# shenyunhang/APE

Measured on AMD Instinct MI355X. Metric: images/sec @1024^2 APE-L_D fwd, higher is better.
Workload: dtype bf16

## Files before the change

ape_amd/_lib.py:

```python
import ctypes
import os
from ctypes import POINTER, Structure, c_char_p, c_double, c_float, c_int, c_int32, c_int64, c_void_p

_HERE = os.path.dirname(os.path.abspath(__file__))
LIB_PATH = os.path.join(_HERE, "lib", "libape_hip.so")

DT_F32 = 0
DT_BF16 = 1
DT_F16 = 2
ACT_NONE, ACT_RELU, ACT_GELU, ACT_SWIGLU, ACT_SILU = 0, 1, 2, 3, 4
MASK_NONE, MASK_ZERO_INPUT, MASK_ZERO_OUTPUT = 0, 1, 2


class GemmArgs(Structure):
    _fields_ = [
        ("A", c_void_p), ("W", c_void_p), ("C", c_void_p), ("bias", c_void_p), ("residual", c_void_p),
        ("rowmask", c_void_p), ("rope_cos", c_void_p), ("rope_sin", c_void_p),
        ("M", c_int32), ("N", c_int32), ("K", c_int32),
        ("lda", c_int32), ("ldw", c_int32), ("ldc", c_int32), ("ldr", c_int32),
        ("in_dt", c_int32), ("out_dt", c_int32), ("res_dt", c_int32),
        ("act", c_int32), ("mask_mode", c_int32), ("trans_out", c_int32),
        ("rope_rows", c_int32), ("rope_hd", c_int32), ("rope_cols", c_int32), ("vec_ok", c_int32),
        ("alpha", c_float), ("clamp", c_float),
        ("splitk", c_int32), ("tile64", c_int32), ("workspace", c_void_p),
        ("rowscale", c_void_p), ("rowshift", c_void_p), ("colvec", c_void_p), ("rope_cs", c_void_p),
        ("ln_w", c_void_p), ("ln_b", c_void_p), ("ln_eps", c_float), ("reserved0", c_int32),
        ("conv_perm", c_void_p), ("conv_zero", c_void_p), ("conv_h", c_int32), ("conv_w", c_int32),
        ("rowstat_cols", c_int32), ("rowstat_eps", c_float),
    ]


class LayerNormArgs(Structure):
    _fields_ = [
        ("x", c_void_p), ("w", c_void_p), ("b", c_void_p), ("y", c_void_p), ("add", c_void_p), ("y2", c_void_p),
        ("M", c_int32), ("C", c_int32), ("Cpad", c_int32),
        ("ldx", c_int32), ("ldy", c_int32), ("ldadd", c_int32), ("ldy2", c_int32),
        ("x_dt", c_int32), ("y_dt", c_int32), ("add_dt", c_int32), ("act", c_int32), ("eps", c_float),
    ]


class GroupNormArgs(Structure):
    _fields_ = [
        ("x", c_void_p), ("w", c_void_p), ("b", c_void_p), ("y", c_void_p), ("add", c_void_p), ("workspace", c_void_p),
        ("HW", c_int32), ("C", c_int32), ("G", c_int32),
        ("ldx", c_int32), ("ldy", c_int32), ("ldadd", c_int32),
        ("x_dt", c_int32), ("y_dt", c_int32), ("add_dt", c_int32), ("act", c_int32), ("eps", c_float),
    ]


SIGNATURES = {
    "ape_hip_last_error": (c_char_p, []),
    "ape_hip_abi_version": (c_int, []),
    "ape_hip_sizeof_args": (c_int, [c_int]),
    "ape_hip_gemm": (c_int, [POINTER(GemmArgs), c_void_p]),
    "ape_hip_gemm_last_kernel": (c_char_p, []),
    "ape_hip_meter_begin": (c_int, []),
    "ape_hip_meter_count": (c_int, []),
    "ape_hip_meter_end": (c_int, []),
    "ape_hip_meter_read": (c_int, [c_int, POINTER(c_char_p), POINTER(c_float)]),
    "ape_hip_zero": (c_int, [c_void_p, ctypes.c_size_t, c_void_p]),
    "ape_hip_stuff_collapse": (c_int, [c_void_p, c_int, c_int, c_int, c_int, c_void_p, c_int, c_void_p]),
    "ape_hip_sem_class_weights": (c_int, [c_void_p, c_int, c_void_p, c_void_p, c_int, c_int, c_int, c_float, c_void_p, c_int, c_int, c_void_p]),
    "ape_hip_pan_class_scores": (c_int, [c_void_p, c_int, c_void_p, c_void_p, c_int, c_int, c_float, c_int, c_float, c_void_p, c_void_p,
                                         c_void_p, c_void_p, c_void_p]),
    "ape_hip_argmax_labels": (c_int, [c_void_p, ctypes.c_size_t, c_int, ctypes.c_size_t, c_float, c_void_p, c_void_p]),
    "ape_hip_sdma_usable": (c_int, [c_void_p, c_void_p]),
    "ape_hip_sdma_d2h": (c_int, [c_void_p, c_void_p, ctypes.c_size_t]),
    "ape_hip_sdma_d2h_multi": (c_int, [c_int, ctypes.POINTER(c_void_p), ctypes.POINTER(c_void_p), ctypes.POINTER(ctypes.c_size_t), c_int]),
    "ape_hip_sdma_engines": (c_int, [c_void_p, c_void_p]),
    "ape_hip_row_stats": (c_int, [c_void_p, c_int, c_int, c_int, c_int, c_float, c_void_p, c_void_p, c_void_p]),
    "ape_hip_gemv": (c_int, [c_void_p, c_int, c_void_p, c_int, c_int, c_void_p, c_void_p, c_int, c_int, c_int, c_int,
                             c_float, c_void_p]),
    "ape_hip_gemv_affine": (c_int, [c_void_p, c_int, c_void_p, c_int, c_int, c_void_p, c_void_p, c_int, c_int, c_int, c_int,
                                    c_float, c_void_p, c_void_p, c_int, c_void_p, c_int, c_void_p]),
    "ape_hip_layernorm": (c_int, [POINTER(LayerNormArgs), c_void_p]),
    "ape_hip_postnorm_residual": (c_int, [c_void_p, c_int, c_int, c_void_p, c_void_p, c_float, c_void_p, c_int, c_void_p, c_int, c_int,
                                          c_int, c_int, c_void_p]),
    "ape_hip_groupnorm_workspace_floats": (c_int, [c_int, c_int]),
    "ape_hip_groupnorm": (c_int, [POINTER(GroupNormArgs), c_void_p]),
    "ape_hip_ms_deform_attn_forward": (c_int, [c_void_p, c_int, POINTER(c_int64), POINTER(c_int64), c_void_p, c_void_p,
                                               c_void_p, c_int, c_int, c_int, c_int, c_int, c_int, c_void_p]),
    "ape_hip_msda_fused": (c_int, [c_void_p, c_int, c_int, POINTER(c_int64), POINTER(c_int64), c_void_p, c_int, c_void_p,
                                   c_int, c_void_p, c_int, c_int, c_int, c_int, c_int, c_int, c_void_p]),
    "ape_hip_msda_fused_h": (c_int, [c_void_p, c_int, c_int, POINTER(c_int64), POINTER(c_int64), c_void_p, c_int, c_void_p,
                                     c_int, c_void_p, c_int, c_int, c_int, c_int, c_int, c_int, c_void_p]),
    "ape_hip_attention": (c_int, [c_void_p, c_int, c_void_p, c_int, c_void_p, c_int, c_void_p, c_int, c_int, c_int, c_int,
                                  c_int, c_float, c_int, c_void_p]),
    "ape_hip_geometry": (c_int, [c_int, c_int, c_int, c_int, POINTER(c_int), c_void_p, c_int, c_void_p, c_float, c_float, c_float,
                                 c_void_p, c_int, c_void_p, c_void_p, c_void_p, c_void_p, c_void_p, c_void_p, c_void_p, c_void_p,
                                 c_void_p]),
    "ape_hip_head_gemv": (c_int, [c_void_p, c_int, c_void_p, c_void_p, c_void_p, c_int, c_int, c_int, c_int, c_float, c_void_p, c_int,
                                  c_int, c_void_p]),
    "ape_hip_attention_strided": (c_int, [c_void_p, c_int, c_void_p, c_int, c_void_p, c_int, c_void_p, c_int, c_int, c_int, c_int,
                                          c_int, c_int, c_float, c_int, c_void_p]),
    "ape_hip_attention_causal": (c_int, [c_void_p, c_int, c_void_p, c_int, c_void_p, c_int, c_void_p, c_int, c_int, c_int, c_int,
                                         c_int, c_int, c_float, c_int, c_void_p]),
    "ape_hip_embed_tokens": (c_int, [c_void_p, c_int, c_void_p, c_int, c_void_p, c_int, c_int, c_void_p, c_int, c_int, c_int, c_int,
                                     c_int, c_int, c_void_p]),
    "ape_hip_patchify": (c_int, [c_void_p, c_int, c_int, c_void_p, c_int, c_int, POINTER(c_float), POINTER(c_float), c_void_p,
                                 c_int, c_int, c_void_p]),
    "ape_hip_im2col3x3": (c_int, [c_void_p, c_int, c_void_p, c_int, c_int, c_int, c_void_p, c_int, c_int, c_void_p]),
    "ape_hip_maxpool2x2": (c_int, [c_void_p, c_int, c_void_p, c_int, c_int, c_int, c_void_p, c_int, c_int, c_void_p]),
    "ape_hip_gather_rows": (c_int, [c_void_p, c_int, c_void_p, c_int, c_int, c_void_p, c_int, c_int, c_void_p]),
    "ape_hip_gather_rows_i64": (c_int, [c_void_p, c_int, c_void_p, c_int, c_int, c_void_p, c_int, c_int, c_void_p]),
    "ape_hip_nms_mask_words": (c_int, [c_int]),
    "ape_hip_nms_mask": (c_int, [c_void_p, c_void_p, c_int, c_float, c_void_p, c_void_p]),
    "ape_hip_nms_scan_segments": (c_int, [c_void_p, c_int, c_void_p, c_int, c_int, c_void_p, c_void_p, c_void_p]),
    "ape_hip_nms_scan_classes": (c_int, [c_void_p, c_int, c_void_p, c_int, c_void_p, c_void_p, c_void_p]),
    "ape_hip_vl_pool_workspace_floats": (c_int, [c_int, c_int]),
    "ape_hip_vl_pool": (c_int, [c_void_p, c_int, c_void_p, c_int, c_int, c_int, c_int, c_void_p, c_void_p, c_void_p, c_void_p]),
    "ape_hip_segment_softmax": (c_int, [c_void_p, c_int, c_int, c_int, c_int, c_void_p, c_void_p, c_int, c_int, c_void_p]),
    "ape_hip_colstats_workspace_floats": (c_int, [c_int, c_int]),
    "ape_hip_colstats": (c_int, [c_void_p, c_int, c_int, c_int, c_void_p, c_void_p, c_void_p, c_void_p, c_void_p]),
    "ape_hip_transpose": (c_int, [c_void_p, c_int, c_int, c_int, c_int, c_void_p, c_void_p, c_void_p, c_void_p, c_int, c_int,
                                  c_void_p]),
    "ape_hip_mask_upsample_bits": (c_int, [c_void_p, c_int, c_int, c_int, c_int, c_int, c_int, c_void_p, c_void_p]),
    "ape_hip_roi_align_bits": (c_int, [c_void_p, c_int, c_int, c_void_p, c_int, c_int, c_void_p, c_void_p]),
    "ape_hip_paste_bits": (c_int, [c_void_p, c_int, c_void_p, c_int, c_int, c_int, c_void_p, c_void_p]),
    "ape_hip_mask_upsample_sigmoid": (c_int, [c_void_p, c_int, c_int, c_int, c_int, c_int, c_int, c_int, c_int, c_void_p, c_int, c_int,
                                              c_void_p]),
    "ape_hip_box_refine": (c_int, [c_void_p, c_int, c_void_p, c_void_p, c_int, c_int, c_float, c_void_p, c_void_p, c_void_p]),
    "ape_hip_det_records": (c_int, [c_void_p, c_void_p, c_void_p, c_void_p, c_void_p, c_int, c_void_p, c_void_p, c_void_p, c_void_p]),
    "ape_hip_query_init": (c_int, [c_void_p, c_void_p, c_int, c_void_p, c_int, c_float, c_int, c_void_p, c_void_p, c_int, c_int, c_void_p,
                                   c_void_p]),
    "ape_hip_query_finish": (c_int, [c_void_p, c_int, c_void_p, c_int, c_int, c_int, c_void_p, c_void_p, c_float, c_void_p, c_void_p,
                                     c_float, c_void_p, c_void_p, c_void_p, c_int, c_int, c_void_p]),
    "ape_hip_bilinear_resize": (c_int, [c_void_p, c_int, c_int, c_int, c_int, c_int, c_void_p, c_int, c_int, c_void_p]),
    "ape_hip_panoptic_pixels": (c_int, [c_void_p, c_int, c_int, c_int, c_int, c_int, c_void_p, c_void_p, c_float, c_int, c_int, c_void_p, c_void_p,
                                        c_void_p, c_void_p]),
    "ape_hip_panoptic_decide": (c_int, [c_void_p, c_void_p, c_void_p, c_int, c_void_p, c_int, c_double, c_int, c_void_p, c_void_p, c_void_p, c_void_p]),
    "ape_hip_panoptic_write": (c_int, [c_void_p, c_void_p, c_void_p, c_int, c_int, c_void_p, c_void_p]),
    "ape_hip_enc_finalize": (c_int, [c_void_p, c_void_p, c_void_p, c_int, c_void_p, c_void_p, c_void_p, c_void_p]),
    "ape_hip_topk_workspace_words": (c_int, [c_int]),
    "ape_hip_proposal_topk": (c_int, [c_void_p, c_int, POINTER(c_int), POINTER(c_int), c_int, c_int, c_int, c_void_p, c_void_p, c_void_p,
                                      c_void_p]),
    "ape_hip_proposal_order": (c_int, [c_void_p, c_int, c_void_p, c_void_p, POINTER(c_int), POINTER(c_int), c_int, c_void_p, c_void_p,
                                       c_void_p, c_void_p, c_void_p, c_void_p, c_void_p]),
    "ape_hip_proposal_quota": (c_int, [c_void_p, c_void_p, c_void_p, c_void_p, c_int, c_void_p, c_int, POINTER(c_int), POINTER(c_int),
                                       c_int, c_int, c_void_p, c_void_p]),
    "ape_hip_det_sort": (c_int, [c_void_p, c_int, c_int, c_int, c_void_p, c_void_p, c_float, c_void_p, c_void_p, c_void_p, c_void_p,
                                 c_void_p, c_void_p]),
    "ape_hip_det_topk": (c_int, [c_void_p, c_void_p, c_void_p, c_void_p, c_int, c_int, c_int, c_void_p, c_void_p, c_void_p, c_void_p,
                                 c_void_p, c_void_p]),
    "ape_hip_ffn_fused": (c_int, [c_void_p, c_int, c_void_p, c_int, c_void_p, c_void_p, c_int, c_void_p, c_void_p, c_int, c_void_p, c_int,
                                  c_int, c_int, c_int, c_int, c_int, c_int, c_void_p, c_void_p, c_float, c_void_p]),
    "ape_hip_attention_ext": (c_int, [c_void_p, c_int, c_void_p, c_int, c_void_p, c_int, c_void_p, c_int, c_int, c_int, c_int, c_int, c_int,
                                      c_int, c_float, c_int, c_void_p]),
    "ape_hip_relpos_extend": (c_int, [c_void_p, c_void_p, c_int, c_void_p, c_int, c_int, c_void_p, c_void_p, c_int, c_void_p, c_void_p, c_int, c_int,
                                      c_int, c_int, c_int, c_int, c_int, c_int, c_float, c_int, c_void_p]),
    "ape_hip_resize_coeffs": (c_int, [c_int, c_int, c_void_p, c_void_p, c_int]),
    "ape_hip_resize_tile_rows": (c_int, [c_void_p, c_int, POINTER(c_int)]),
    "ape_hip_resize_bilinear_u8": (c_int, [c_void_p, c_int, c_int, c_int, c_void_p, c_void_p, c_int, c_void_p, c_void_p, c_int,
                                           c_int, c_int, c_int, c_int, c_void_p, c_int, c_int, c_int, c_int, c_void_p]),
    "ape_hip_rle_workspace_words": (c_int, [c_int, c_int, c_int, c_int]),
    "ape_hip_rle_encode": (c_int, [c_void_p, c_int, c_int, c_int, c_void_p, c_void_p, c_int, c_void_p, c_void_p]),
    "ape_hip_rle_to_string": (c_int, [c_void_p, c_int, c_void_p, c_int]),
    "ape_hip_label_hist_lds_bins": (c_int, []),
    "ape_hip_label_pair_hist": (c_int, [c_void_p, c_int, c_void_p, c_int, ctypes.c_size_t, c_int, c_int, c_int, c_int, c_void_p, c_void_p,
                                        c_void_p]),
    "ape_hip_mask_pack_bits": (c_int, [c_void_p, c_int, ctypes.c_size_t, ctypes.c_size_t, c_void_p, ctypes.c_size_t, c_void_p, c_void_p]),
    "ape_hip_mask_paired_counts": (c_int, [c_void_p, ctypes.c_size_t, c_void_p, ctypes.c_size_t, c_int, ctypes.c_size_t, c_void_p, c_void_p]),
    "ape_hip_bitmask_pair_counts": (c_int, [c_void_p, c_int, ctypes.c_size_t, c_void_p, c_int, ctypes.c_size_t, ctypes.c_size_t, c_void_p,
                                            ctypes.c_size_t, c_void_p]),
    "ape_hip_rle_decode_workspace_words": (c_int, [c_int, c_int]),
    "ape_hip_rle_decode": (c_int, [c_void_p, c_void_p, c_int, c_int, c_int, c_int, c_void_p, c_void_p, c_void_p]),
    "ape_hip_rle_from_string": (c_int, [c_void_p, c_int, c_void_p, c_int]),
    "ape_hip_mask_pack_rows": (c_int, [c_void_p, c_int, c_int, c_int, c_void_p, ctypes.c_size_t, c_void_p, c_void_p]),
    "ape_hip_bitmask_boundary": (c_int, [c_void_p, c_int, c_int, c_int, c_int, ctypes.c_size_t, c_void_p, ctypes.c_size_t, c_void_p,
                                         c_void_p]),
    "ape_hip_bitmask_boundary_tile": (c_int, [c_int, c_int, c_int, ctypes.c_size_t, POINTER(c_int), POINTER(c_int)]),
    "ape_hip_bitmask_unpack_rows": (c_int, [c_void_p, c_int, c_int, c_int, ctypes.c_size_t, c_void_p, c_void_p]),
    "ape_hip_box_cover_overlaps": (c_int, [c_void_p, c_int, c_void_p, c_void_p, c_int, c_void_p, c_void_p, c_int, c_void_p, c_void_p,
                                           c_void_p]),
    "ape_hip_coco_match": (c_int, [c_void_p, c_int, c_int, ctypes.c_size_t, c_void_p, c_int, c_void_p, c_void_p, c_int, c_void_p, c_int,
                                   c_void_p, c_void_p, c_void_p, c_void_p, c_int, c_void_p, c_int, c_void_p, c_void_p, c_void_p]),
}

_lib = None


def load():
    global _lib
    if _lib is not None:
        return _lib
    if not os.path.exists(LIB_PATH):
        raise RuntimeError(
            f"{LIB_PATH} not found: the HIP extension is not built (run `python -m ape_amd.build` or "
            "__graft_entry__.build()).  ape_amd has no CPU/PyTorch fallback."
        )
    lib = ctypes.CDLL(LIB_PATH)
    for name, (res, args) in SIGNATURES.items():
        fn = getattr(lib, name)
        fn.restype = res
        fn.argtypes = args
    _lib = lib
    return lib


def check(rc, what):
    if rc != 0:
        msg = load().ape_hip_last_error()
        raise RuntimeError(f"{what} failed (rc={rc}): {msg.decode() if msg else '?'}")
```

ape_amd/csrc/boxes.hip:

```cpp
#include "common.h"
#include "../../include/ape_hip.h"

__global__ __launch_bounds__(256) void box_refine_kernel(const float* __restrict__ delta, int ldd, const float* __restrict__ ref,
                                                         const float* __restrict__ vr4, int L, int Q, float eps,
                                                         float* __restrict__ new_ref, float* __restrict__ ref_in) {
  const int gid = blockIdx.x * 256 + threadIdx.x;
  if (gid >= Q * 4) return;
  const int q = gid >> 2, c = gid & 3;
  float x = ref[gid];
  x = fminf(fmaxf(x, 0.f), 1.f);
  const float x1 = fmaxf(x, eps), x2 = fmaxf(1.f - x, eps);
  float z = logf(x1 / x2);
  if (delta != nullptr) z += delta[(size_t)q * ldd + c];
  const float r = delta != nullptr ? 1.f / (1.f + expf(-z)) : ref[gid];
  if (new_ref != nullptr) new_ref[gid] = r;
  if (ref_in != nullptr)
    for (int l = 0; l < L; ++l) ref_in[((size_t)q * L + l) * 4 + c] = r * vr4[l * 4 + c];
}

extern "C" int ape_hip_box_refine(const float* delta, int ldd, const float* ref, const float* vr4, int L, int Q, float eps,
                                  float* new_ref, float* ref_in, void* stream) {
  APE_CHECK_ARG(ref && Q > 0 && (ref_in == nullptr || (vr4 != nullptr && L > 0)) && (new_ref || ref_in),
                "ape_hip_box_refine: bad args");
  APE_LAUNCH(box_refine_kernel, dim3(ceil_div(Q * 4, 256)), dim3(256), 0, (hipStream_t)stream, delta, ldd, ref, vr4, L, Q, eps,
                     new_ref, ref_in);
  APE_CHECK_LAUNCH("ape_hip_box_refine");
  return 0;
}

template <typename T> __device__ __forceinline__ float round_to(float v);
template <> __device__ __forceinline__ float round_to<float>(float v) { return v; }
template <> __device__ __forceinline__ float round_to<bf16_t>(float v) { return bf2f(f2bf(v)); }
template <> __device__ __forceinline__ float round_to<f16_t>(float v) { return (float)(f16_t)sat_h(v); }

template <typename TO>
__global__ __launch_bounds__(256) void query_init_kernel(const float* __restrict__ coords, const int64_t* __restrict__ topk, int T,
                                                         const float* __restrict__ dim_t, int P, float scale, int Q,
                                                         float* __restrict__ reference, TO* __restrict__ pe, int ldpe,
                                                         int32_t* __restrict__ topk32) {
  const int q = blockIdx.x;
  int64_t t = topk[q];
  t = t < 0 ? 0 : (t >= T ? T - 1 : t);
  if (threadIdx.x == 0 && topk32 != nullptr) topk32[q] = (int32_t)t;
  for (int j = threadIdx.x; j < 4 * P; j += 256) {
    const int c = j / P, i = j % P;
    const float x = coords[(size_t)t * 4 + c];
    const float s = 1.f / (1.f + expf(-x));
    if (i == 0) reference[q * 4 + c] = s;
    const float v = (s * scale) / dim_t[i];
    stf<TO>(pe + (size_t)q * ldpe + j, (i & 1) ? cosf(v) : sinf(v));
  }
}

extern "C" int ape_hip_query_init(const float* coords, const int64_t* topk, int T, const float* dim_t, int P, float scale, int Q,
                                  float* reference, void* pe, int ldpe, int pe_dt, int32_t* topk32, void* stream) {
  APE_CHECK_ARG(coords && topk && dim_t && reference && pe && T > 0 && P > 0 && Q > 0 && ldpe >= 4 * P, "ape_hip_query_init: bad args");
  hipStream_t s = (hipStream_t)stream;
  if (pe_dt == APE_DT_F16) APE_LAUNCH(query_init_kernel<f16_t>, dim3(Q), dim3(256), 0, s, coords, topk, T, dim_t, P, scale, Q, reference, (f16_t*)pe, ldpe, topk32);
  else if (pe_dt == APE_DT_BF16) APE_LAUNCH(query_init_kernel<bf16_t>, dim3(Q), dim3(256), 0, s, coords, topk, T, dim_t, P, scale, Q, reference, (bf16_t*)pe, ldpe, topk32);
  else if (pe_dt == APE_DT_F32)
    APE_LAUNCH(query_init_kernel<float>, dim3(Q), dim3(256), 0, s, coords, topk, T, dim_t, P, scale, Q, reference, (float*)pe, ldpe, topk32);
  else
    APE_CHECK_ARG(false, "ape_hip_query_init: pe must be f32, bf16 or f16");
  APE_CHECK_LAUNCH("ape_hip_query_init");
  return 0;
}

template <typename TO>
__global__ __launch_bounds__(256) void query_finish_kernel(const float* __restrict__ pos, int ldpos, const float* __restrict__ pix,
                                                           int ldpix, int Q, int E, const float* __restrict__ wpos,
                                                           const float* __restrict__ bpos, float eps_pos,
                                                           const float* __restrict__ wpix, const float* __restrict__ bpix,
                                                           float eps_pix, TO* __restrict__ query_pos, TO* __restrict__ query,
                                                           TO* __restrict__ query_sum, int ldo) {
  const int lane = threadIdx.x & 63;
  const int q = blockIdx.x * 4 + (threadIdx.x >> 6);
  if (q >= Q) return;
  constexpr int MAXP = 16, MAXX = 8;
  float vp[MAXP], vx[MAXX];
  const float* pr = pos + (size_t)q * ldpos;
  const float* xr = pix + (size_t)q * ldpix;
  float sp = 0.f, sx = 0.f;
#pragma unroll
  for (int k = 0; k < MAXP; ++k) { const int c = lane + 64 * k; vp[k] = c < 2 * E ? pr[c] : 0.f; sp += vp[k]; }
#pragma unroll
  for (int k = 0; k < MAXX; ++k) { const int c = lane + 64 * k; vx[k] = c < E ? xr[c] : 0.f; sx += vx[k]; }
  const float mp = wave_sum(sp) / (float)(2 * E), mx = wave_sum(sx) / (float)E;
  float qp = 0.f, qx = 0.f;
#pragma unroll
  for (int k = 0; k < MAXP; ++k) { const int c = lane + 64 * k; const float d = c < 2 * E ? vp[k] - mp : 0.f; qp += d * d; }
#pragma unroll
  for (int k = 0; k < MAXX; ++k) { const int c = lane + 64 * k; const float d = c < E ? vx[k] - mx : 0.f; qx += d * d; }
  const float rp = rsqrtf(wave_sum(qp) / (float)(2 * E) + eps_pos), rx = rsqrtf(wave_sum(qx) / (float)E + eps_pix);
  const int kE = E / 64;
#pragma unroll
  for (int k = 0; k < MAXX; ++k) {
    const int c = lane + 64 * k;
    if (c < E) {
      const float a = (vp[k] - mp) * rp * wpos[c] + bpos[c];
      float hi = 0.f;
#pragma unroll
      for (int kk = 0; kk < MAXP; ++kk) if (kk == k + kE) hi = (vp[kk] - mp) * rp * wpos[E + c] + bpos[E + c];
      const float b = hi + ((vx[k] - mx) * rx * wpix[c] + bpix[c]);
      const float ar = round_to<TO>(a), br = round_to<TO>(b);
      stf<TO>(query_pos + (size_t)q * ldo + c, ar);
      stf<TO>(query + (size_t)q * ldo + c, br);
      stf<TO>(query_sum + (size_t)q * ldo + c, ar + br);
    }
  }
}

extern "C" int ape_hip_query_finish(const float* pos, int ldpos, const float* pix, int ldpix, int Q, int E, const float* wpos,
                                    const float* bpos, float eps_pos, const float* wpix, const float* bpix, float eps_pix,
                                    void* query_pos, void* query, void* query_sum, int ldo, int out_dt, void* stream) {
  APE_CHECK_ARG(pos && pix && wpos && bpos && wpix && bpix && query_pos && query && query_sum && Q > 0, "ape_hip_query_finish: bad args");
  APE_CHECK_ARG(E > 0 && E <= 512 && E % 64 == 0 && ldpos >= 2 * E && ldpix >= E && ldo >= E, "ape_hip_query_finish: E must be a multiple of 64, <= 512");
  hipStream_t s = (hipStream_t)stream;
  const dim3 grid(ceil_div(Q, 4)), block(256);
  if (out_dt == APE_DT_F16) APE_LAUNCH(query_finish_kernel<f16_t>, grid, block, 0, s, pos, ldpos, pix, ldpix, Q, E, wpos, bpos, eps_pos, wpix, bpix, eps_pix,
                       (f16_t*)query_pos, (f16_t*)query, (f16_t*)query_sum, ldo);
  else if (out_dt == APE_DT_BF16) APE_LAUNCH(query_finish_kernel<bf16_t>, grid, block, 0, s, pos, ldpos, pix, ldpix, Q, E, wpos, bpos, eps_pos, wpix, bpix, eps_pix,
                       (bf16_t*)query_pos, (bf16_t*)query, (bf16_t*)query_sum, ldo);
  else if (out_dt == APE_DT_F32)
    APE_LAUNCH(query_finish_kernel<float>, grid, block, 0, s, pos, ldpos, pix, ldpix, Q, E, wpos, bpos, eps_pos, wpix, bpix, eps_pix,
                       (float*)query_pos, (float*)query, (float*)query_sum, ldo);
  else
    APE_CHECK_ARG(false, "ape_hip_query_finish: outputs must be f32, bf16 or f16");
  APE_CHECK_LAUNCH("ape_hip_query_finish");
  return 0;
}

__global__ __launch_bounds__(1024) void det_records_kernel(const float* __restrict__ boxes, const float* __restrict__ scores,
                                                            const int64_t* __restrict__ classes, const int64_t* __restrict__ query,
                                                            const float* __restrict__ frame, int k, float* __restrict__ rec,
                                                            float* __restrict__ boxes_out, int32_t* __restrict__ order) {
  __shared__ int wtot[16];
  __shared__ int total_keep;
  const int tid = threadIdx.x, lane = tid & 63, wave = tid >> 6;
  float f[8];
#pragma unroll
  for (int i = 0; i < 8; ++i) f[i] = frame[i];
  int cnt = 0;
  for (int i = tid; i < k; i += 1024) {
    float b[4];
#pragma unroll
    for (int c = 0; c < 4; ++c) b[c] = fminf(fmaxf(boxes[i * 4 + c] * f[c], 0.f), f[4 + c]);
    cnt += (scores[i] >= 0.f && (b[2] - b[0]) > 0.f && (b[3] - b[1]) > 0.f) ? 1 : 0;
  }
  cnt = (int)wave_sum((float)cnt);
  if (lane == 0) wtot[wave] = cnt;
  __syncthreads();
  if (tid == 0) { int s = 0; for (int w = 0; w < 16; ++w) s += wtot[w]; total_keep = s; }
  __syncthreads();
  int kbase = 0, dbase = total_keep;
  for (int i0 = 0; i0 < k; i0 += 1024) {
    const int i = i0 + tid;
    const bool in = i < k;
    float b[4] = {0.f, 0.f, 0.f, 0.f};
    bool keep = false;
    float sc = -1.f;
    if (in) {
#pragma unroll
      for (int c = 0; c < 4; ++c) b[c] = fminf(fmaxf(boxes[i * 4 + c] * f[c], 0.f), f[4 + c]);
      sc = scores[i];
      keep = sc >= 0.f && (b[2] - b[0]) > 0.f && (b[3] - b[1]) > 0.f;
    }
    const unsigned long long m = __ballot(keep);
    const int before = __popcll(m & ((1ull << lane) - 1ull));
    __syncthreads();
    if (lane == 0) wtot[wave] = __popcll(m);
    __syncthreads();
    int wbase = 0, chunk_keep = 0;
    for (int w = 0; w < 16; ++w) { const int t = wtot[w]; if (w < wave) wbase += t; chunk_keep += t; }
    if (in) {
      const int kept_before = wbase + before;
      const int pos = keep ? kbase + kept_before : dbase + (tid - kept_before);
      float* r = rec + (size_t)pos * 8;
      r[0] = b[0]; r[1] = b[1]; r[2] = b[2]; r[3] = b[3];
      r[4] = keep ? sc : -1.f;
      r[5] = (float)classes[i];
      r[6] = (float)query[i];
      r[7] = keep ? 1.f : 0.f;
      float* bo = boxes_out + (size_t)pos * 4;
      bo[0] = b[0]; bo[1] = b[1]; bo[2] = b[2]; bo[3] = b[3];
      order[pos] = i;
    }
    const int nin = min(1024, k - i0);
    kbase += chunk_keep;
    dbase += nin - chunk_keep;
  }
}

extern "C" int ape_hip_det_records(const float* boxes, const float* scores, const int64_t* classes, const int64_t* query,
                                   const float* frame, int k, float* rec, float* boxes_out, int32_t* order, void* stream) {
  APE_CHECK_ARG(boxes && scores && classes && query && frame && rec && boxes_out && order && k > 0, "ape_hip_det_records: bad args");
  APE_LAUNCH(det_records_kernel, dim3(1), dim3(1024), 0, (hipStream_t)stream, boxes, scores, classes, query, frame, k, rec,
                     boxes_out, order);
  APE_CHECK_LAUNCH("ape_hip_det_records");
  return 0;
}
```

ape_amd/csrc/norm.hip:

```cpp
#include "common.h"
#include "../../include/ape_hip.h"

__device__ __forceinline__ float ln_act(float x, int act) {
  if (act == APE_ACT_RELU) return fmaxf(x, 0.f);
  if (act == APE_ACT_GELU) return 0.5f * x * (1.f + erff(x * 0.70710678118654752440f));
  return x;
}

template <typename TX, typename TY, typename TA, int NV4>
__global__ __launch_bounds__(256) void layernorm_kernel(const ApeLayerNormArgs p) {
  const int lane = threadIdx.x & 63;
  const int row = blockIdx.x * 4 + (threadIdx.x >> 6);
  if (row >= p.M) return;
  const TX* x = reinterpret_cast<const TX*>(p.x) + (size_t)row * p.ldx;
  TY* y = reinterpret_cast<TY*>(p.y) + (size_t)row * p.ldy;
  const TA* add = p.add ? reinterpret_cast<const TA*>(p.add) + (size_t)row * p.ldadd : nullptr;
  TY* y2 = p.y2 ? reinterpret_cast<TY*>(p.y2) + (size_t)row * p.ldy2 : nullptr;
  const int C = p.C;
  const float invC = 1.f / (float)C;
  float v[NV4][4];
  float s = 0.f;
#pragma unroll
  for (int i = 0; i < NV4; ++i) {
    const int c = (i * 64 + lane) * 4;
    if (c + 3 < C) {
      ld4<TX>(x + c, v[i]);
    } else {
#pragma unroll
      for (int r = 0; r < 4; ++r) v[i][r] = (c + r < C) ? ldf<TX>(x + c + r) : 0.f;
    }
    s += (v[i][0] + v[i][1]) + (v[i][2] + v[i][3]);
  }
  const float mean = wave_sum(s) * invC;
  float q = 0.f;
#pragma unroll
  for (int i = 0; i < NV4; ++i) {
    const int c = (i * 64 + lane) * 4;
#pragma unroll
    for (int r = 0; r < 4; ++r) {
      const float d = (c + r < C) ? v[i][r] - mean : 0.f;
      q = fmaf(d, d, q);
    }
  }
  const float rstd = rsqrtf(wave_sum(q) * invC + p.eps);
#pragma unroll
  for (int i = 0; i < NV4; ++i) {
    const int c = (i * 64 + lane) * 4;
    if (c >= p.Cpad) continue;
    float o[4], o2[4];
    if (c + 3 < C) {
      float w4[4], b4[4];
      ld4<float>(p.w + c, w4);
      ld4<float>(p.b + c, b4);
#pragma unroll
      for (int r = 0; r < 4; ++r) o[r] = ln_act((v[i][r] - mean) * rstd * w4[r] + b4[r], p.act);
      st4<TY>(y + c, o);
      if (y2 != nullptr) {
        ld4<TA>(add + c, o2);
#pragma unroll
        for (int r = 0; r < 4; ++r) o2[r] += o[r];
        st4<TY>(y2 + c, o2);
      }
      continue;
    }
#pragma unroll
    for (int r = 0; r < 4; ++r) {
      if (c + r < C) {
        o[r] = ln_act((v[i][r] - mean) * rstd * p.w[c + r] + p.b[c + r], p.act);
        o2[r] = (y2 != nullptr) ? o[r] + ldf<TA>(add + c + r) : 0.f;
      } else {
        o[r] = 0.f; o2[r] = 0.f;
      }
    }
    if (c + 3 < p.Cpad) {
      st4<TY>(y + c, o);
      if (y2 != nullptr) st4<TY>(y2 + c, o2);
    } else {
      for (int r = 0; r < 4 && c + r < p.Cpad; ++r) { stf<TY>(y + c + r, o[r]); if (y2 != nullptr) stf<TY>(y2 + c + r, o2[r]); }
    }
  }
  for (int c = NV4 * 256 + lane; c < p.Cpad; c += 64) { stf<TY>(y + c, 0.f); if (y2 != nullptr) stf<TY>(y2 + c, 0.f); }
}

template <typename TX, typename TY, typename TA>
__global__ __launch_bounds__(256) void layernorm_generic_kernel(const ApeLayerNormArgs p) {
  const int lane = threadIdx.x & 63;
  const int row = blockIdx.x * 4 + (threadIdx.x >> 6);
  if (row >= p.M) return;
  const TX* x = reinterpret_cast<const TX*>(p.x) + (size_t)row * p.ldx;
  TY* y = reinterpret_cast<TY*>(p.y) + (size_t)row * p.ldy;
  const TA* add = p.add ? reinterpret_cast<const TA*>(p.add) + (size_t)row * p.ldadd : nullptr;
  TY* y2 = p.y2 ? reinterpret_cast<TY*>(p.y2) + (size_t)row * p.ldy2 : nullptr;
  const int C = p.C;
  const float invC = 1.f / (float)C;
  float s = 0.f;
  for (int c = lane; c < C; c += 64) s += ldf<TX>(x + c);
  const float mean = wave_sum(s) * invC;
  float q = 0.f;
  for (int c = lane; c < C; c += 64) { const float d = ldf<TX>(x + c) - mean; q = fmaf(d, d, q); }
  const float rstd = rsqrtf(wave_sum(q) * invC + p.eps);
  for (int c = lane; c < C; c += 64) {
    const float o = ln_act((ldf<TX>(x + c) - mean) * rstd * p.w[c] + p.b[c], p.act);
    stf<TY>(y + c, o);
    if (y2 != nullptr) stf<TY>(y2 + c, o + ldf<TA>(add + c));
  }
  for (int c = C + lane; c < p.Cpad; c += 64) {
    stf<TY>(y + c, 0.f);
    if (y2 != nullptr) stf<TY>(y2 + c, 0.f);
  }
}

template <typename TX, typename TY, typename TA>
static int launch_ln(const ApeLayerNormArgs& p, hipStream_t s) {
  const dim3 grid(ceil_div(p.M, 4)), block(256);
  const bool vec = (p.ldx % 4 == 0) && (p.ldy % 4 == 0) && (((uintptr_t)p.x) % 16 == 0) && (((uintptr_t)p.y) % 16 == 0) &&
                   (((uintptr_t)p.w) % 16 == 0) && (((uintptr_t)p.b) % 16 == 0) &&
                   (!p.y2 || ((p.ldadd % 4 == 0) && (p.ldy2 % 4 == 0) && (((uintptr_t)p.add) % 16 == 0) &&
                              (((uintptr_t)p.y2) % 16 == 0)));
  const int need = p.Cpad > p.C ? p.Cpad : p.C;
  if (vec && need <= 256) APE_LAUNCH((layernorm_kernel<TX, TY, TA, 1>), grid, block, 0, s, p);
  else if (vec && need <= 512) APE_LAUNCH((layernorm_kernel<TX, TY, TA, 2>), grid, block, 0, s, p);
  else if (vec && need <= 1024) APE_LAUNCH((layernorm_kernel<TX, TY, TA, 4>), grid, block, 0, s, p);
  else if (vec && need <= 2048) APE_LAUNCH((layernorm_kernel<TX, TY, TA, 8>), grid, block, 0, s, p);
  else if (vec && need <= 3072) APE_LAUNCH((layernorm_kernel<TX, TY, TA, 12>), grid, block, 0, s, p);
  else APE_LAUNCH((layernorm_generic_kernel<TX, TY, TA>), grid, block, 0, s, p);
  return 0;
}

extern "C" int ape_hip_layernorm(const ApeLayerNormArgs* a, void* stream) {
  APE_CHECK_ARG(a && a->x && a->y && a->w && a->b, "ape_hip_layernorm: null pointer");
  APE_CHECK_ARG(a->M > 0 && a->C > 0 && a->Cpad >= a->C, "ape_hip_layernorm: bad shape");
  APE_CHECK_ARG((a->add == nullptr) == (a->y2 == nullptr), "ape_hip_layernorm: add and y2 go together");
  const ApeLayerNormArgs p = *a;
  hipStream_t s = (hipStream_t)stream;
  const int add_dt = p.add ? p.add_dt : p.y_dt;
  const int hk = APE_H16_KIND(p.x_dt, p.y_dt, add_dt);
  if (hk < 0) { ape_set_error("ape_hip_layernorm: dtypes must be f32 or ONE 16-bit type (x %d, y %d, add %d)", p.x_dt, p.y_dt, add_dt); return -1; }
  const int key = (ape_is16(p.x_dt) ? 4 : 0) + (ape_is16(p.y_dt) ? 2 : 0) + (ape_is16(add_dt) ? 1 : 0);
#define APE_NORM_CASES(H_)                                      \
  switch (key) {                                                \
    case 0: launch_ln<float, float, float>(p, s); break;        \
    case 1: launch_ln<float, float, H_>(p, s); break;           \
    case 2: launch_ln<float, H_, float>(p, s); break;           \
    case 3: launch_ln<float, H_, H_>(p, s); break;              \
    case 4: launch_ln<H_, float, float>(p, s); break;           \
    case 5: launch_ln<H_, float, H_>(p, s); break;              \
    case 6: launch_ln<H_, H_, float>(p, s); break;              \
    default: launch_ln<H_, H_, H_>(p, s); break;                \
  }
  if (hk == APE_DT_F16) { APE_NORM_CASES(f16_t) } else { APE_NORM_CASES(bf16_t) }
#undef APE_NORM_CASES
  APE_CHECK_LAUNCH("ape_hip_layernorm");
  return 0;
}

#define GN_ROWS_PER_BLOCK 128

template <typename TX>
__global__ __launch_bounds__(256) void gn_partial_kernel(const TX* __restrict__ x, int ldx, int HW, int C, int G,
                                                         float* __restrict__ partial) {
  __shared__ float sh[8 * 256 + 256];
  __shared__ float smean[64];
  const int t = threadIdx.x;
  const int cg = C / G;
  const int r0 = blockIdx.x * GN_ROWS_PER_BLOCK;
  const int r1 = min(r0 + GN_ROWS_PER_BLOCK, HW);
  const int nrows = r1 - r0;
  const bool vec = (C % 8 == 0) && (256 % (C / 8) == 0) && (256 / (C / 8) <= 8) && (ldx % 8 == 0) && (((uintptr_t)x) % 16 == 0);
  const int ncg = vec ? C / 8 : 0, nrl = vec ? 256 / ncg : 0;
  const int cgi = vec ? t % ncg : 0, rl = vec ? t / ncg : 0;
  float* tot = sh + 8 * 256;
  for (int pass = 0; pass < 2; ++pass) {
    if (vec) {
      float a[8];
      float mu[8];
#pragma unroll
      for (int c = 0; c < 8; ++c) { a[c] = 0.f; mu[c] = pass ? smean[(cgi * 8 + c) / cg] : 0.f; }
      for (int r = r0 + rl; r < r1; r += nrl) {
        float v[8];
        ld8<TX>(x + (size_t)r * ldx + cgi * 8, v);
#pragma unroll
        for (int c = 0; c < 8; ++c) { const float d = v[c] - mu[c]; a[c] += pass ? d * d : d; }
      }
#pragma unroll
      for (int c = 0; c < 8; ++c) sh[rl * 256 + cgi * 8 + c] = a[c];
      __syncthreads();
      if (t < C) {
        float z = 0.f;
        for (int k = 0; k < nrl; ++k) z += sh[k * 256 + t];
        tot[t] = z;
      }
    } else {
      float z = 0.f;
      if (t < C) {
        const float m = pass ? smean[t / cg] : 0.f;
        for (int r = r0; r < r1; ++r) { const float d = ldf<TX>(x + (size_t)r * ldx + t) - m; z += pass ? d * d : d; }
      }
      tot[t] = z;
    }
    __syncthreads();
    if (t < G) {
      float z = 0.f;
      for (int j = 0; j < cg; ++j) z += tot[t * cg + j];
      if (pass == 0) smean[t] = z / (float)(nrows * cg);
      else {
        partial[((size_t)blockIdx.x * G + t) * 2 + 0] = smean[t];
        partial[((size_t)blockIdx.x * G + t) * 2 + 1] = z;
      }
    }
    __syncthreads();
  }
}

__global__ __launch_bounds__(64) void gn_finalize_kernel(const float* __restrict__ partial, int nchunk, int HW, int cg,
                                                         int G, float eps, float* __restrict__ stats) {
  const int g = blockIdx.x, lane = threadIdx.x;
  float n = 0.f, mean = 0.f, m2 = 0.f;
  for (int k = lane; k < nchunk; k += 64) {
    const int rows = min(GN_ROWS_PER_BLOCK, HW - k * GN_ROWS_PER_BLOCK);
    const float nb = (float)(rows * cg);
    const float mb = partial[((size_t)k * G + g) * 2 + 0];
    const float qb = partial[((size_t)k * G + g) * 2 + 1];
    const float nt = n + nb;
    const float delta = mb - mean;
    mean += delta * (nb / nt);
    m2 += qb + delta * delta * (n * nb / nt);
    n = nt;
  }
#pragma unroll
  for (int o = 32; o > 0; o >>= 1) {
    const float nb = __shfl_xor(n, o, 64), mb = __shfl_xor(mean, o, 64), qb = __shfl_xor(m2, o, 64);
    const float nt = n + nb;
    if (nt > 0.f) {
      const float delta = mb - mean;
      mean = (n * mean + nb * mb) / nt;
      m2 = m2 + qb + delta * delta * (n * nb / nt);
    }
    n = nt;
  }
  if (lane == 0) {
    stats[g * 2 + 0] = mean;
    stats[g * 2 + 1] = rsqrtf(m2 / n + eps);
  }
}

template <typename TX, typename TY, typename TA>
__global__ __launch_bounds__(256) void gn_apply_kernel(const TX* __restrict__ x, int ldx, int HW, int C, int G,
                                                       const float* __restrict__ stats, const float* __restrict__ w,
                                                       const float* __restrict__ b, int act, const TA* __restrict__ add,
                                                       int ldadd, TY* __restrict__ y, int ldy) {
  const int t = threadIdx.x;
  const int cg = C / G;
  const int r0 = blockIdx.x * GN_ROWS_PER_BLOCK;
  const int r1 = min(r0 + GN_ROWS_PER_BLOCK, HW);
  const bool vec = (C % 8 == 0) && (256 % (C / 8) == 0) && (ldx % 8 == 0) && (ldy % 8 == 0) && (((uintptr_t)x) % 16 == 0) &&
                   (((uintptr_t)y) % 16 == 0) && (add == nullptr || (ldadd % 8 == 0 && ((uintptr_t)add) % 16 == 0));
  if (vec) {
    const int ncg = C / 8, nrl = 256 / ncg;
    const int cgi = t % ncg, rl = t / ncg;
    float wt[8], bt[8];
#pragma unroll
    for (int c = 0; c < 8; ++c) {
      const int ch = cgi * 8 + c;
      const float m = stats[(ch / cg) * 2 + 0], rs = stats[(ch / cg) * 2 + 1];
      wt[c] = w[ch] * rs; bt[c] = b[ch] - m * rs * w[ch];
    }
    for (int r = r0 + rl; r < r1; r += nrl) {
      float v[8];
      ld8<TX>(x + (size_t)r * ldx + cgi * 8, v);
#pragma unroll
      for (int c = 0; c < 8; ++c) v[c] = fmaf(v[c], wt[c], bt[c]);
      if (add != nullptr) {
        float av[8];
        ld8<TA>(add + (size_t)r * ldadd + cgi * 8, av);
#pragma unroll
        for (int c = 0; c < 8; ++c) v[c] += av[c];
      }
      if (act == APE_ACT_RELU) {
#pragma unroll
        for (int c = 0; c < 8; ++c) v[c] = fmaxf(v[c], 0.f);
      }
      st8<TY>(y + (size_t)r * ldy + cgi * 8, v);
    }
    return;
  }
  if (t >= C) return;
  const float m = stats[(t / cg) * 2 + 0], rs = stats[(t / cg) * 2 + 1];
  const float wt = w[t] * rs, bt = b[t] - m * rs * w[t];
  for (int r = r0; r < r1; ++r) {
    float v = fmaf(ldf<TX>(x + (size_t)r * ldx + t), wt, bt);
    if (add != nullptr) v += ldf<TA>(add + (size_t)r * ldadd + t);
    if (act == APE_ACT_RELU) v = fmaxf(v, 0.f);
    stf<TY>(y + (size_t)r * ldy + t, v);
  }
}

template <typename TX, typename TY, typename TA>
static void launch_gn(const ApeGroupNormArgs& p, hipStream_t s) {
  const int nchunk = ceil_div(p.HW, GN_ROWS_PER_BLOCK);
  float* stats = p.workspace + (size_t)nchunk * p.G * 2;
  APE_LAUNCH((gn_partial_kernel<TX>), dim3(nchunk), dim3(256), 0, s, (const TX*)p.x, p.ldx, p.HW, p.C, p.G,
                     p.workspace);
  APE_LAUNCH(gn_finalize_kernel, dim3(p.G), dim3(64), 0, s, p.workspace, nchunk, p.HW, p.C / p.G, p.G, p.eps, stats);
  APE_LAUNCH((gn_apply_kernel<TX, TY, TA>), dim3(nchunk), dim3(256), 0, s, (const TX*)p.x, p.ldx, p.HW, p.C, p.G,
                     stats, p.w, p.b, p.act, (const TA*)p.add, p.ldadd, (TY*)p.y, p.ldy);
}

extern "C" int ape_hip_groupnorm_workspace_floats(int HW, int G) { return ceil_div(HW, GN_ROWS_PER_BLOCK) * G * 2 + G * 2; }

extern "C" int ape_hip_groupnorm(const ApeGroupNormArgs* a, void* stream) {
  APE_CHECK_ARG(a && a->x && a->y && a->w && a->b && a->workspace, "ape_hip_groupnorm: null pointer");
  APE_CHECK_ARG(a->C > 0 && a->C <= 256 && a->G > 0 && a->G <= 64 && a->C % a->G == 0 && a->HW > 0,
                "ape_hip_groupnorm: need C <= 256, G <= 64, C %% G == 0");
  const ApeGroupNormArgs p = *a;
  hipStream_t s = (hipStream_t)stream;
  const int add_dt = p.add ? p.add_dt : p.y_dt;
  const int hk = APE_H16_KIND(p.x_dt, p.y_dt, add_dt);
  if (hk < 0) { ape_set_error("ape_hip_groupnorm: dtypes must be f32 or ONE 16-bit type (x %d, y %d, add %d)", p.x_dt, p.y_dt, add_dt); return -1; }
  const int key = (ape_is16(p.x_dt) ? 4 : 0) + (ape_is16(p.y_dt) ? 2 : 0) + (ape_is16(add_dt) ? 1 : 0);
#define APE_NORM_CASES(H_)                                      \
  switch (key) {                                                \
    case 0: launch_gn<float, float, float>(p, s); break;        \
    case 1: launch_gn<float, float, H_>(p, s); break;           \
    case 2: launch_gn<float, H_, float>(p, s); break;           \
    case 3: launch_gn<float, H_, H_>(p, s); break;              \
    case 4: launch_gn<H_, float, float>(p, s); break;           \
    case 5: launch_gn<H_, float, H_>(p, s); break;              \
    case 6: launch_gn<H_, H_, float>(p, s); break;              \
    default: launch_gn<H_, H_, H_>(p, s); break;                \
  }
  if (hk == APE_DT_F16) { APE_NORM_CASES(f16_t) } else { APE_NORM_CASES(bf16_t) }
#undef APE_NORM_CASES
  APE_CHECK_LAUNCH("ape_hip_groupnorm");
  return 0;
}


template <typename TX>
__global__ __launch_bounds__(256) void row_stats_kernel(const TX* __restrict__ x, int ldx, int M, int C, float eps,
                                                        float* __restrict__ rowscale, float* __restrict__ rowshift) {
  const int lane = threadIdx.x & 63;
  const int row = blockIdx.x * 4 + (threadIdx.x >> 6);
  if (row >= M) return;
  const TX* xr = x + (size_t)row * ldx;
  const int C8 = (ldx % 8 == 0 && ((uintptr_t)x) % 16 == 0) ? (C & ~7) : 0;
  float s = 0.f;
  for (int c = lane * 8; c < C8; c += 512) {
    float v[8];
    ld8<TX>(xr + c, v);
    s += ((v[0] + v[1]) + (v[2] + v[3])) + ((v[4] + v[5]) + (v[6] + v[7]));
  }
  for (int c = C8 + lane; c < C; c += 64) s += ldf<TX>(xr + c);
  const float mean = wave_sum(s) / (float)C;
  float q = 0.f;
  for (int c = lane * 8; c < C8; c += 512) {
    float v[8];
    ld8<TX>(xr + c, v);
#pragma unroll
    for (int i = 0; i < 8; ++i) { const float d = v[i] - mean; q = fmaf(d, d, q); }
  }
  for (int c = C8 + lane; c < C; c += 64) { const float d = ldf<TX>(xr + c) - mean; q = fmaf(d, d, q); }
  const float rstd = rsqrtf(wave_sum(q) / (float)C + eps);
  if (lane == 0) { rowscale[row] = rstd; rowshift[row] = -mean * rstd; }
}

extern "C" int ape_hip_row_stats(const void* x, int ldx, int dt, int M, int C, float eps, float* rowscale, float* rowshift,
                                 void* stream) {
  APE_CHECK_ARG(x && rowscale && rowshift && M > 0 && C > 0, "ape_hip_row_stats: bad args");
  const dim3 grid(ceil_div(M, 4)), block(256);
  if (dt == APE_DT_F16) APE_LAUNCH(row_stats_kernel<f16_t>, grid, block, 0, (hipStream_t)stream, (const f16_t*)x, ldx, M, C, eps, rowscale, rowshift);
  else if (dt == APE_DT_BF16) APE_LAUNCH(row_stats_kernel<bf16_t>, grid, block, 0, (hipStream_t)stream, (const bf16_t*)x, ldx, M, C, eps, rowscale, rowshift);
  else APE_LAUNCH(row_stats_kernel<float>, grid, block, 0, (hipStream_t)stream, (const float*)x, ldx, M, C, eps, rowscale, rowshift);
  APE_CHECK_LAUNCH("ape_hip_row_stats");
  return 0;
}

template <typename TT, typename TC, int NV4>
__global__ __launch_bounds__(256) void postnorm_residual_kernel(const TT* __restrict__ t, int ldt, const float* __restrict__ w,
                                                                const float* __restrict__ b, float eps, float* __restrict__ stream,
                                                                int lds, TC* __restrict__ copy, int ldc, int M, int C) {
  const int lane = threadIdx.x & 63;
  const int row = blockIdx.x * 4 + (threadIdx.x >> 6);
  if (row >= M) return;
  float* xs = stream + (size_t)row * lds;
// ... 78 lines not shown
```

ape_amd/layers/multi_scale_deform_attn.py:

```python
import os

import torch
import torch.nn as nn

from .. import ops
from ..packing import attach_cache, f32, pack_matrix


def multi_scale_deformable_attn_pytorch(value, value_spatial_shapes, sampling_locations, attention_weights):
    shapes = [(int(h), int(w)) for h, w in (value_spatial_shapes.tolist() if torch.is_tensor(value_spatial_shapes) else value_spatial_shapes)]
    starts = [0]
    for h, w in shapes[:-1]:
        starts.append(starts[-1] + h * w)
    return ops.ms_deform_attn_forward(value.contiguous(), shapes, starts, sampling_locations.to(value.dtype).contiguous(),
                                      attention_weights.to(value.dtype).contiguous())


def _register_torch_op():
    try:
        lib = torch.library.Library("ape", "DEF")
        lib.define("ms_deform_attn_forward(Tensor value, Tensor spatial_shapes, Tensor level_start_index, "
                   "Tensor sampling_loc, Tensor attn_weight, int im2col_step) -> Tensor")

        def impl(value, spatial_shapes, level_start_index, sampling_loc, attn_weight, im2col_step):
            return ops.ms_deform_attn_forward(value, spatial_shapes, level_start_index, sampling_loc, attn_weight, im2col_step)

        lib.impl("ms_deform_attn_forward", impl, "CUDA")
        return lib
    except RuntimeError as exc:
        if "ms_deform_attn_forward" in str(exc) and hasattr(torch.ops.ape, "ms_deform_attn_forward"):
            return None
        raise


_TORCH_LIB = _register_torch_op()


HALF_MAX = 65504.0


def half_value_kwargs(dt, rows):
    if dt == torch.bfloat16 and rows >= 2048 and os.environ.get("APE_MSDA_BF16_VALUE") != "1":
        return dict(out_dtype=torch.float16)
    return {}


class MultiScaleDeformableAttention(nn.Module):
    def __init__(self, embed_dim=256, num_heads=8, num_levels=4, num_points=4, img2col_step=64, dropout=0.1,
                 batch_first=False, pytorch_attn=False):
        super().__init__()
        if embed_dim != 256 or num_heads != 8 or num_points != 4:
            raise ValueError("ape_amd MSDeformAttn kernel is built for embed_dim=256, 8 heads, 4 points (APE configs)")
        self.dropout = nn.Dropout(dropout)
        self.batch_first = batch_first
        self.im2col_step = img2col_step
        self.embed_dim, self.num_heads, self.num_levels, self.num_points = embed_dim, num_heads, num_levels, num_points
        self.sampling_offsets = nn.Linear(embed_dim, num_heads * num_levels * num_points * 2)
        self.attention_weights = nn.Linear(embed_dim, num_heads * num_levels * num_points)
        self.value_proj = nn.Linear(embed_dim, embed_dim)
        self.output_proj = nn.Linear(embed_dim, embed_dim)
        self.pytorch_attn = pytorch_attn
        self.compute_dtype = torch.bfloat16
        attach_cache(self)

    def packed(self, dt):
        def build(dt):
            w = torch.cat([self.sampling_offsets.weight, self.attention_weights.weight], 0).detach()
            b = torch.cat([self.sampling_offsets.bias.detach().float(), self.attention_weights.bias.detach().float()])
            n, npad = w.shape[0], -(-w.shape[0] // 128) * 128
            if npad != n:
                w = torch.cat([w, w.new_zeros((npad - n, w.shape[1]))], 0)
                b = torch.cat([b, b.new_zeros((npad - n,))])
            return dict(
                woffw=pack_matrix(w, dt), boffw=b.contiguous(), noffw=n,
                wval=pack_matrix(self.value_proj.weight, dt), bval=f32(self.value_proj.bias),
                wout=pack_matrix(self.output_proj.weight, dt), bout=f32(self.output_proj.bias))
        return self._pack.get(self, dt, build)

    def forward_tokens(self, query_pos_sum, identity, ref, shapes, starts, dt, *, value_src=None, value=None, mask=None,
                       out_dtype=None, norm=None):
        P = self.packed(dt)
        if value is None:
            value = ops.gemm(value_src, P["wval"], P["bval"], rowmask=mask, mask_mode=ops.MASK_ZERO_OUTPUT,
                             **half_value_kwargs(dt, value_src.shape[0]))
        half = dt in ops.HALF16 and query_pos_sum.shape[0] >= 2048 and os.environ.get("APE_MSDA_F32_OFFSETS") != "1"
        offw = ops.gemm(query_pos_sum, P["woffw"], P["boffw"], out_dtype=torch.float16 if half else torch.float32)[:, :P["noffw"]]
        samp = ops.msda_fused(value, shapes, starts, offw, ref, out_dtype=dt)
        if norm is not None and ops.gemm_norm_fusable(samp, P["wout"], identity, out_dtype):
            return ops.gemm(samp, P["wout"], P["bout"], residual=identity, norm=norm)
        y = ops.gemm(samp, P["wout"], P["bout"], residual=identity, out_dtype=out_dtype or dt)
        return y if norm is None else ops.layernorm(y, norm[0], norm[1], norm[2], out_dtype=out_dtype or dt)

    def forward(self, query, key=None, value=None, identity=None, query_pos=None, key_padding_mask=None,
                reference_points=None, spatial_shapes=None, level_start_index=None, **kwargs):
        if value is None:
            value = query
        if identity is None:
            identity = query
        if query_pos is not None:
            query = query + query_pos
        if not self.batch_first:
            query, value, identity_b = query.permute(1, 0, 2), value.permute(1, 0, 2), identity.permute(1, 0, 2)
        else:
            identity_b = identity
        bs, nq, _ = query.shape
        shapes = [(int(h), int(w)) for h, w in spatial_shapes.tolist()]
        assert sum(h * w for h, w in shapes) == value.shape[1]
        starts = [0]
        for h, w in shapes[:-1]:
            starts.append(starts[-1] + h * w)
        dt = self.compute_dtype
        outs = []
        for b in range(bs):
            m = key_padding_mask[b].to(torch.uint8).contiguous() if key_padding_mask is not None else None
            o = self.forward_tokens(query[b].to(dt).contiguous(), identity_b[b].to(dt).contiguous(),
                                    reference_points[b].float().contiguous(), shapes, starts, dt,
                                    value_src=value[b].to(dt).contiguous(), mask=m)
            outs.append(o.to(identity.dtype))
        out = torch.stack(outs)
        if not self.batch_first:
            out = out.permute(1, 0, 2)
        return out
```

ape_amd/modeling/ape_deta/_containers.py:

```python
import os

import torch
import torch.nn as nn

from ... import ops
from ...packing import attach_cache, f32, ln_params, pack_matrix, permute_ffn_w2


class FFN(nn.Module):
    def __init__(self, embed_dim=256, feedforward_dim=1024, output_dim=None, num_fcs=2, ffn_drop=0.0, **kwargs):
        super().__init__()
        assert num_fcs == 2
        output_dim = embed_dim if output_dim is None else output_dim
        self.layers = nn.Sequential(nn.Sequential(nn.Linear(embed_dim, feedforward_dim), nn.ReLU(inplace=True), nn.Dropout(ffn_drop)),
                                    nn.Linear(feedforward_dim, output_dim), nn.Dropout(ffn_drop))
        self.embed_dim = embed_dim
        attach_cache(self)

    def packed(self, dt):
        def build(dt):
            l0, l1 = self.layers[0][0], self.layers[1]
            d = dict(w1=pack_matrix(l0.weight, dt), b1=f32(l0.bias), w2=pack_matrix(l1.weight, dt), b2=f32(l1.bias))
            if dt in ops.HALF16 and l0.weight.shape[0] % 64 == 0:
                d["w2p"] = permute_ffn_w2(d["w2"])
            return d
        return self._pack.get(self, dt, build)

    FUSED_MIN_ROWS = 2048

    def forward_tokens(self, x, dt, out_dtype=None, norm=None):
        P = self.packed(dt)
        mode = os.environ.get("APE_FFN_FUSED", "1")
        if (mode != "0" and "w2p" in P and (out_dtype or dt) in ops.HALF16 and (out_dtype or dt) == dt and x.shape[0] >= self.FUSED_MIN_ROWS
                and x.shape[1] == 256 and P["w2"].shape[0] == 256 and P["w1"].shape[0] <= 4096):
            fuse_ln = norm if os.environ.get("APE_FFN_LN") != "0" else None
            if mode == "b64":
                y = ops.ffn_fused(x, P["w1"], P["b1"], P["w2"], P["b2"], residual=x, norm=fuse_ln)
            else:
                y = ops.ffn_fused(x, P["w1"], P["b1"], P["w2p"], P["b2"], residual=x, w2_permuted=True, norm=fuse_ln)
            return y if (norm is None or fuse_ln is not None) else ops.layernorm(y, norm[0], norm[1], norm[2], out_dtype=dt)
        h = ops.gemm(x, P["w1"], P["b1"], act=ops.ACT_RELU)
        y = ops.gemm(h, P["w2"], P["b2"], residual=x, out_dtype=out_dtype or dt)
        return y if norm is None else ops.layernorm(y, norm[0], norm[1], norm[2], out_dtype=dt)


class MLP(nn.Module):
    def __init__(self, input_dim, hidden_dim, output_dim, num_layers):
        super().__init__()
        self.num_layers = num_layers
        h = [hidden_dim] * (num_layers - 1)
        self.layers = nn.ModuleList(nn.Linear(n, k) for n, k in zip([input_dim] + h, h + [output_dim]))
        attach_cache(self)

    def packed(self, dt):
        def build(dt):
            return [(pack_matrix(l.weight, dt), f32(l.bias)) for l in self.layers]
        return self._pack.get(self, dt, build)

    def forward_tokens(self, x, dt, out_dtype=torch.float32):
        P = self.packed(dt)
        for i, (w, b) in enumerate(P):
            last = i == len(P) - 1
            x = ops.gemm(x, w, b, act=ops.ACT_NONE if last else ops.ACT_RELU, out_dtype=out_dtype if last else dt)
        return x


class SelfAttention(nn.Module):

    def __init__(self, embed_dim, num_heads, attn_drop=0.0, proj_drop=0.0, batch_first=False, **kwargs):
        super().__init__()
        self.embed_dim, self.num_heads, self.batch_first = embed_dim, num_heads, batch_first
        self.attn = nn.MultiheadAttention(embed_dim=embed_dim, num_heads=num_heads, dropout=attn_drop, batch_first=batch_first)
        self.proj_drop = nn.Dropout(proj_drop)
        attach_cache(self)

    def packed(self, dt):
        def build(dt):
            E = self.embed_dim
            w, b = self.attn.in_proj_weight, self.attn.in_proj_bias
            return dict(wqk=pack_matrix(w[:2 * E], dt), bqk=f32(b[:2 * E]), wv=pack_matrix(w[2 * E:], dt), bv=f32(b[2 * E:]),
                        wo=pack_matrix(self.attn.out_proj.weight, dt), bo=f32(self.attn.out_proj.bias))
        return self._pack.get(self, dt, build)

    def forward_tokens(self, x, x_pos, dt, vt_buf, out_dtype=None):
        P = self.packed(dt)
        E, nh = self.embed_dim, self.num_heads
        hd = E // nh
        vjob = ops.fork(lambda: ops.gemm(x, P["wv"], P["bv"], trans_out=True, out=vt_buf))
        qk = ops.gemm(x_pos, P["wqk"], P["bqk"])
        vt = vjob.join()
        o = ops.attention(qk[:, :E], qk[:, E:], vt, batch=1, n=x.shape[0], heads=nh, head_dim=hd, scale=hd ** -0.5)
        return ops.gemm(o, P["wo"], P["bo"], residual=x, out_dtype=out_dtype or dt)


class TransformerLayer(nn.Module):

    def __init__(self, attentions, ffn, num_norms, embed_dim=256):
        super().__init__()
        self.attentions = nn.ModuleList(attentions)
        self.ffns = nn.ModuleList([ffn])
        self.norms = nn.ModuleList([nn.LayerNorm(embed_dim) for _ in range(num_norms)])
        self.embed_dim = embed_dim
        self.pre_norm = False

    def norm_params(self, i):
        return ln_params(self.norms[i])


class ConvNormAct(nn.Module):
    def __init__(self, in_channels, out_channels, kernel_size=1, bias=True, norm_layer=None):
        super().__init__()
        self.conv = nn.Conv2d(in_channels, out_channels, kernel_size=kernel_size, padding=(kernel_size - 1) // 2, bias=bias)
        self.norm = norm_layer


class ChannelMapper(nn.Module):

    def __init__(self, input_shapes, in_features, out_channels, kernel_size=1, stride=1, bias=True, groups=1, dilation=1,
                 norm_layer=None, activation=None, num_outs=None, **kwargs):
        super().__init__()
        import copy
        assert kernel_size == 1 and activation is None
        chans = [getattr(input_shapes[f], "channels", input_shapes[f]) for f in in_features]
        assert num_outs is None or num_outs == len(chans), "extra downsampling convs are not used by the APE configs"
        self.convs = nn.ModuleList(ConvNormAct(c, out_channels, 1, bias, copy.deepcopy(norm_layer)) for c in chans)
        self.in_features, self.out_channels, self.input_shapes = in_features, out_channels, input_shapes


class PositionEmbeddingSine(nn.Module):

    def __init__(self, num_pos_feats=64, temperature=10000, scale=2 * 3.141592653589793, eps=1e-6, offset=0.0, normalize=False):
        super().__init__()
        self.num_pos_feats, self.temperature, self.scale, self.eps, self.offset, self.normalize = (
            num_pos_feats, temperature, scale, eps, offset, normalize)
```

ape_amd/modeling/ape_deta/deformable_transformer_vl.py:

```python
import copy

import torch
import torch.nn as nn

from ... import ops
from ...layers import MultiScaleDeformableAttention
from ...packing import attach_cache, f32, ln_params, pack_matrix, round_up
from ...stagetap import forcing, tap
from . import geometry as G
from ._containers import FFN, SelfAttention, TransformerLayer


class DeformableDetrTransformerEncoderVL(nn.Module):
    def __init__(self, embed_dim=256, num_heads=8, feedforward_dim=1024, attn_dropout=0.1, ffn_dropout=0.1, num_layers=6,
                 post_norm=False, num_feature_levels=4, vl_layer=None, use_act_checkpoint=False, pytorch_attn=False):
        super().__init__()
        self.layers = nn.ModuleList([
            TransformerLayer([MultiScaleDeformableAttention(embed_dim=embed_dim, num_heads=num_heads, dropout=attn_dropout,
                                                            batch_first=True, num_levels=num_feature_levels,
                                                            pytorch_attn=pytorch_attn)],
                             FFN(embed_dim=embed_dim, feedforward_dim=feedforward_dim, output_dim=embed_dim, num_fcs=2,
                                 ffn_drop=ffn_dropout), 2, embed_dim) for _ in range(num_layers)])
        self.num_layers = num_layers
        self.embed_dim = embed_dim
        self.pre_norm = False
        self.post_norm_layer = nn.LayerNorm(embed_dim) if post_norm else None
        self.vl_layers = nn.ModuleList([copy.deepcopy(vl_layer) for _ in range(num_layers)]) if vl_layer is not None else None
        self.use_checkpoint = use_act_checkpoint

    def forward_tokens(self, x, geo, lvl_pos, l, dt, stages=None):
        xp = None
        for i, layer in enumerate(self.layers):
            if self.vl_layers is None:
                v_new, qp, ljob = x, (xp if xp is not None else (x.float() + lvl_pos.float()).to(dt)), ops._Joined(l)
            else:
                v_new, qp, ljob = self.vl_layers[i].b_attn.forward_tokens(x, lvl_pos, l, dt, defer_language=True)
            x2 = layer.attentions[0].forward_tokens(qp, v_new, geo.enc_ref, geo.shapes, geo.starts, dt, value_src=v_new,
                                                    mask=geo.mask_u8, norm=layer.norm_params(0))
            x, xp = layer.ffns[0].forward_tokens(x2, dt, norm=layer.norm_params(1)), None
            l = ljob.join()
            if stages is not None:
                if self.vl_layers is not None:
                    stages[f"enc{i}_fused_v"] = v_new
                    l = tap(stages, f"enc{i}_fused_l", l)
                x = tap(stages, f"enc{i}_out", x)
        if self.post_norm_layer is not None:
            x = ops.layernorm(x, *ln_params(self.post_norm_layer), out_dtype=dt)
        return x, l


class DeformableDetrTransformerDecoderVL(nn.Module):
    def __init__(self, embed_dim=256, num_heads=8, feedforward_dim=1024, attn_dropout=0.1, ffn_dropout=0.1, num_layers=6,
                 return_intermediate=True, num_feature_levels=4, use_act_checkpoint=False, look_forward_twice=False,
                 pytorch_attn=False):
        super().__init__()
        self.layers = nn.ModuleList([
            TransformerLayer([SelfAttention(embed_dim=embed_dim, num_heads=num_heads, attn_drop=attn_dropout, batch_first=True),
                              MultiScaleDeformableAttention(embed_dim=embed_dim, num_heads=num_heads, dropout=attn_dropout,
                                                            batch_first=True, num_levels=num_feature_levels,
                                                            pytorch_attn=pytorch_attn)],
                             FFN(embed_dim=embed_dim, feedforward_dim=feedforward_dim, output_dim=embed_dim, ffn_drop=ffn_dropout),
                             3, embed_dim) for _ in range(num_layers)])
        self.num_layers = num_layers
        self.embed_dim = embed_dim
        self.return_intermediate = return_intermediate
        self.bbox_embed = None
        self.class_embed = None
        self.use_checkpoint = use_act_checkpoint
        self.look_forward_twice = look_forward_twice
        attach_cache(self)

    def packed(self, dt):
        def build(dt):
            ws = [l.attentions[1].value_proj.weight for l in self.layers]
            bs = [l.attentions[1].value_proj.bias.detach().float() for l in self.layers]
            return dict(wval=pack_matrix(torch.cat(ws, 0), dt), bval=torch.cat(bs).contiguous())
        return self._pack.get(self, dt, build)

    def forward_tokens(self, query, query_pos, memory, geo, reference, dt, stages=None, query_sum=None):
        P = self.packed(dt)
        E = self.embed_dim
        from ...layers.multi_scale_deform_attn import half_value_kwargs
        value_all = ops.gemm(memory, P["wval"], P["bval"], rowmask=geo.mask_u8, mask_mode=ops.MASK_ZERO_OUTPUT,
                             **half_value_kwargs(dt, memory.shape[0]))
        Q = query.shape[0]
        vt_buf = ops.zeros((E, round_up(Q, 64)), dt, query.device)
        vr4 = geo.vr4
        out = query
        outp = query_sum if query_sum is not None else (query.float() + query_pos.float()).to(dt)
        inter, inter_ref = [], []
        _, ref_in = ops.box_refine(None, reference.contiguous(), vr4)
        refjob = ops._Joined((reference, ref_in))
        for i, layer in enumerate(self.layers):
            x1 = layer.attentions[0].forward_tokens(out, outp, dt, vt_buf)
            x2, x2p = ops.layernorm(x1, *layer.norm_params(0), out_dtype=dt, add=query_pos)
            reference, ref_in = refjob.join()
            if i > 0:
                if stages is not None:
                    forced = tap(stages, f"dec{i - 1}_ref", reference)
                    if forced is not reference:
                        reference = forced
                        _, ref_in = ops.box_refine(None, reference.contiguous(), vr4)
                inter_ref.append(reference)
            x3 = layer.attentions[1].forward_tokens(x2p, x2, ref_in, geo.shapes, geo.starts, dt,
                                                    value=value_all[:, i * E:(i + 1) * E])
            x4 = ops.layernorm(x3, *layer.norm_params(1), out_dtype=dt)
            x5 = layer.ffns[0].forward_tokens(x4, dt)
            out, outp = ops.layernorm(x5, *layer.norm_params(2), out_dtype=dt, add=query_pos)
            if stages is not None:
                forced = tap(stages, f"dec{i}_out", out)
                if forced is not out:
                    out, outp = forced, (forced.float() + query_pos.float()).to(dt)
            if self.bbox_embed is not None:
                def refine(i=i, out=out, reference=reference):
                    tmp = self.bbox_embed[i].forward_tokens(out, dt, out_dtype=torch.float32)
                    if stages is not None:
                        stages[f"dec{i}_delta"] = tmp
                    return ops.box_refine(tmp, reference, vr4)
                refjob = ops.fork(refine)
            inter.append(out)
        reference, _ = refjob.join()
        reference = tap(stages, f"dec{len(self.layers) - 1}_ref", reference)
        inter_ref.append(reference)
        return inter, inter_ref


class DeformableDetrTransformerVL(nn.Module):
    def __init__(self, encoder=None, decoder=None, num_feature_levels=4, as_two_stage=False, two_stage_num_proposals=300,
                 assign_first_stage=False, pre_nms_topk=1000, nms_thresh_enc=0.9, proposal_ambiguous=0):
        super().__init__()
        assert as_two_stage and assign_first_stage, "ape_amd implements the two-stage DETA selection used by every APE config"
        self.encoder, self.decoder = encoder, decoder
        self.num_feature_levels = num_feature_levels
        self.as_two_stage = as_two_stage
        self.two_stage_num_proposals = two_stage_num_proposals
        self.assign_first_stage = assign_first_stage
        self.pre_nms_topk, self.nms_thresh_enc = pre_nms_topk, nms_thresh_enc
        self.proposal_ambiguous = proposal_ambiguous
        self.compute_dtype = torch.bfloat16
        self.embed_dim = self.encoder.embed_dim
        self.level_embeds = nn.Parameter(torch.Tensor(self.num_feature_levels, self.embed_dim))
        self.enc_output = nn.Linear(self.embed_dim, self.embed_dim)
        self.enc_output_norm = nn.LayerNorm(self.embed_dim)
        self.pos_trans = nn.Linear(self.embed_dim * 2, self.embed_dim * 2)
        self.pos_trans_norm = nn.LayerNorm(self.embed_dim * 2)
        self.pix_trans = nn.Linear(self.embed_dim, self.embed_dim)
        self.pix_trans_norm = nn.LayerNorm(self.embed_dim)
        nn.init.normal_(self.level_embeds)
        attach_cache(self)

    def packed(self, dt):
        def build(dt):
            dec = self.decoder
            nd = dec.num_layers
            amb = bool(self.proposal_ambiguous)
            be, bea = dec.bbox_embed[nd], (dec.bbox_embed_ambiguous[0] if amb else dec.bbox_embed[nd])
            ce, cea = dec.class_embed[nd], (dec.class_embed_ambiguous[0] if amb else dec.class_embed[nd])
            return dict(
                wenc=pack_matrix(self.enc_output.weight, dt), benc=f32(self.enc_output.bias),
                nenc=ln_params(self.enc_output_norm),
                wpos=pack_matrix(self.pos_trans.weight, dt), bpos=f32(self.pos_trans.bias),
                npos=ln_params(self.pos_trans_norm),
                wpix=pack_matrix(self.pix_trans.weight, dt), bpix=f32(self.pix_trans.bias),
                npix=ln_params(self.pix_trans_norm),
                w1=pack_matrix(torch.cat([be.layers[0].weight, bea.layers[0].weight], 0), dt),
                b1=torch.cat([be.layers[0].bias, bea.layers[0].bias]).detach().float().contiguous(),
                w2=(pack_matrix(be.layers[1].weight, dt), pack_matrix(bea.layers[1].weight, dt)),
                b2=(f32(be.layers[1].bias), f32(bea.layers[1].bias)),
                w3=(pack_matrix(be.layers[2].weight, dt), pack_matrix(bea.layers[2].weight, dt)),
                b3=(f32(be.layers[2].bias), f32(bea.layers[2].bias)),
                wcls=pack_matrix(torch.cat([ce.weight, cea.weight], 0), dt),
                bcls=torch.cat([ce.bias, cea.bias]).detach().float().contiguous(),
                level_embeds=f32(self.level_embeds))
        return self._pack.get(self, dt, build)

    def lvl_pos(self, geo, dt):
        key = (dt, self.level_embeds.data_ptr(), self.level_embeds._version)
        if key not in geo._lvl_pos:
            geo._lvl_pos.clear()
            geo._lvl_pos[key] = (geo.pos + self.level_embeds.detach().float()[geo.level_ids]).to(dt).contiguous()
        return geo._lvl_pos[key]

    def forward_tokens(self, src, geo, l, dt, forced_topk=None, stages=None, after_encoder=None, mask_prompt=None):
        P = self.packed(dt)
        lvl_pos = self.lvl_pos(geo, dt)
        memory, l_out = self.encoder.forward_tokens(src, geo, lvl_pos, l, dt, stages)
        memory = tap(stages, "memory", memory)
        if after_encoder is not None:
            after_encoder(memory)
        invalid, anchors = geo.invalid_u8, geo.proposals
        if mask_prompt is not None:
            outside = ~mask_prompt.reshape(-1).to(device=memory.device, dtype=torch.bool)
            invalid = (invalid.reshape(-1).bool() | outside).to(torch.uint8).reshape(invalid.shape).contiguous()
            anchors = anchors.masked_fill(outside[:, None], float("inf")).contiguous()
        om = ops.gemm(memory, P["wenc"], P["benc"], rowmask=invalid, mask_mode=ops.MASK_ZERO_INPUT)
        om = tap(stages, "output_memory", ops.layernorm(om, *P["nenc"], out_dtype=dt))
        E = self.embed_dim
        T = om.shape[0]
        h1 = ops.gemm(om, P["w1"], P["b1"], act=ops.ACT_RELU)
        h2 = torch.empty((T, 2 * E), dtype=dt, device=om.device)
        ops.gemm(h1[:, :E], P["w2"][0], P["b2"][0], act=ops.ACT_RELU, out=h2[:, :E])
        ops.gemm(h1[:, E:], P["w2"][1], P["b2"][1], act=ops.ACT_RELU, out=h2[:, E:])
        d = torch.empty((T, 8), dtype=torch.float32, device=om.device)
        ops.gemm(h2[:, :E], P["w3"][0], P["b3"][0], out=d[:, :4])
        ops.gemm(h2[:, E:], P["w3"][1], P["b3"][1], out=d[:, 4:])
        cls2 = ops.gemm(om, P["wcls"], P["bcls"], out_dtype=torch.float32)
        if stages is not None:
            cls2, d = tap(stages, "enc_cls2", cls2), tap(stages, "enc_delta8", d)
        enc_class, enc_coord, xyxy = ops.enc_finalize(cls2, d, anchors)
        if stages is not None:
            stages["query_l"] = l_out
            enc_class, enc_coord = tap(stages, "enc_class", enc_class), tap(stages, "enc_coord_unact", enc_coord)
        if forced_topk is not None:
            topk = forced_topk.to(om.device).long()
        else:
            topk = ops.select_proposals(enc_class, xyxy, geo.shapes, self.pre_nms_topk, self.two_stage_num_proposals,
                                        self.nms_thresh_enc)
        reference, pe, topk32 = ops.query_init(enc_coord, topk, G.dim_t_table(128, 10000, om.device), dt)
        pos_raw = ops.gemm(pe, P["wpos"], P["bpos"], out_dtype=torch.float32)
        pix_raw = ops.gemm(ops.gather_rows(om, topk32), P["wpix"], P["bpix"], out_dtype=torch.float32)
        query_pos, query, query_sum = ops.query_finish(pos_raw, pix_raw, P["npos"], P["npix"], dt)
        if stages is not None:
            stages["topk_proposals"] = topk
            q0, p0 = query, query_pos
            query, query_pos = tap(stages, "query_init", query), tap(stages, "query_pos", query_pos)
            if query is not q0 or query_pos is not p0:
                query_sum = None
            reference = tap(stages, "init_reference", reference)
        inter, inter_ref = self.decoder.forward_tokens(query, query_pos, memory, geo, reference, dt, stages, query_sum=query_sum)
        return dict(inter_states=inter, init_reference=reference, inter_references=inter_ref, enc_class=enc_class,
                    enc_coord_unact=enc_coord, memory=memory, query_l=l_out, topk_proposals=topk)

    def forward(self, multi_level_feats, multi_level_masks, multi_level_pos_embeds, query_embed=None, query_l=None, attention_mask_l=None,
                multi_level_masks_prompt=None, **kwargs):
        if not self.as_two_stage or query_embed is not None:
            raise NotImplementedError("ape_amd: the two-stage transformer of the APE configs (as_two_stage=True, no query_embed)")
        if attention_mask_l is not None:
            raise NotImplementedError("ape_amd: language masks (un-reduced text tokens, text_feature_reduce_before_fusion=False) are not implemented")
        dt = getattr(self, "compute_dtype", torch.bfloat16)
        B = multi_level_feats[0].shape[0]
        rows = []
        for b in range(B):
            masks = [m[b].bool() for m in multi_level_masks]
            pos = [p[b].flatten(1).t() for p in multi_level_pos_embeds]
            geo = G.geometry_from_masks(masks, pos)
            src = torch.cat([f[b].flatten(1).t() for f in multi_level_feats]).to(dt).contiguous()
            mp = None if multi_level_masks_prompt is None else torch.cat([m[b].reshape(-1) for m in multi_level_masks_prompt]).to(torch.bool)
            tr = self.forward_tokens(src, geo, query_l[b].float().contiguous(), dt, mask_prompt=mp)
            anchors = geo.proposals if mp is None else geo.proposals.masked_fill(~mp.to(geo.proposals.device)[:, None], float("inf"))
            rows.append((torch.stack(tr["inter_states"]), tr["init_reference"], torch.stack(tr["inter_references"]),
                         tr["enc_class"][:, None], tr["enc_coord_unact"], anchors.sigmoid(), tr["memory"], tr["query_l"]))
        odt = multi_level_feats[0].dtype
        cat = lambda i, dim: torch.stack([r[i] for r in rows], dim)
        return (cat(0, 1).to(odt), cat(1, 0).to(odt), cat(2, 1).to(odt), cat(3, 0).to(odt), cat(4, 0).to(odt), cat(5, 0).to(odt),
                cat(6, 0).to(odt), cat(7, 0).to(query_l.dtype))
```

ape_amd/ops.py:

```python
import ctypes
import math
import os

import numpy as np
import torch

from . import _lib
from ._lib import (ACT_GELU, ACT_NONE, ACT_RELU, ACT_SILU, ACT_SWIGLU, DT_BF16, DT_F32, MASK_NONE,
                   MASK_ZERO_INPUT, MASK_ZERO_OUTPUT)

_DT = {torch.float32: DT_F32, torch.bfloat16: DT_BF16, torch.float16: _lib.DT_F16}
HALF16 = (torch.bfloat16, torch.float16)


def _dt(t):
    try:
        return _DT[t.dtype]
    except KeyError:
        raise TypeError(f"ape_amd: unsupported dtype {t.dtype} (float32 / bfloat16 / float16 only)")


def _dev(*ts):
    for t in ts:
        if t is not None and not t.is_cuda:
# ... 502 lines not shown
    _lib.check(rc, "ape_hip_gather_rows")
    return out


def _boxes(b):
    if b.dtype != torch.float32 or not b.is_contiguous() or b.dim() != 2 or b.shape[1] != 4:
        raise ValueError("ape_amd.ops: boxes must be contiguous float32 [n,4]")
    return b


def _u8(t, name):
    if t is None:
        return None
    if t.dtype not in (torch.uint8, torch.bool) or not t.is_contiguous():
        raise ValueError(f"ape_amd.ops: {name} must be contiguous uint8/bool")
    return t


def nms_segments(boxes, groups, seg_offsets, max_segment, iou_thr, valid=None):
    _dev(boxes, groups, seg_offsets, valid)
    n = boxes.shape[0]
    lib = _lib.load()
    mask = torch.empty((n, lib.ape_hip_nms_mask_words(n)), dtype=torch.int64, device=boxes.device)
    keep = torch.zeros((n,), dtype=torch.uint8, device=boxes.device)
    _lib.check(lib.ape_hip_nms_mask(_p(_boxes(boxes)), _p(_i32(groups, "groups")), n, float(iou_thr), _p(mask), _stream()), "ape_hip_nms_mask")
    rc = lib.ape_hip_nms_scan_segments(_p(mask), n, _p(_i32(seg_offsets, "seg_offsets")), seg_offsets.numel() - 1, int(max_segment),
                                       _p(_u8(valid, "valid")), _p(keep), _stream())
    _lib.check(rc, "ape_hip_nms_scan_segments")
    return keep


def nms_classes(boxes, order, iou_thr, valid=None):
    _dev(boxes, order, valid)
    n = boxes.shape[0]
    K = order.shape[0]
    lib = _lib.load()
    mask = torch.empty((n, lib.ape_hip_nms_mask_words(n)), dtype=torch.int64, device=boxes.device)
    keep = torch.zeros((K, n), dtype=torch.uint8, device=boxes.device)
    _lib.check(lib.ape_hip_nms_mask(_p(_boxes(boxes)), None, n, float(iou_thr), _p(mask), _stream()), "ape_hip_nms_mask")
    rc = lib.ape_hip_nms_scan_classes(_p(mask), n, _p(_i32(order, "order")), K, _p(_u8(valid, "valid")), _p(keep), _stream())
    _lib.check(rc, "ape_hip_nms_scan_classes")
    return keep


def vl_pool(scores, x, sub=None):
    _dev(scores, x, sub)
    _rowmajor(scores, "scores"), _rowmajor(x, "x")
    if scores.dtype != torch.float32 or scores.shape[1] != 8:
        raise ValueError("ape_amd.ops.vl_pool: scores must be float32 [T,8]")
    T, C = x.shape
    if sub is not None and sub.numel() != C:
        raise ValueError("ape_amd.ops.vl_pool: sub must have one entry per channel")
    lib = _lib.load()
    ws = torch.empty((lib.ape_hip_vl_pool_workspace_floats(T, C),), dtype=torch.float32, device=x.device)
    out = torch.empty((8, C), dtype=torch.float32, device=x.device)
    rc = lib.ape_hip_vl_pool(_p(scores), _ld(scores), _p(x), _ld(x), _dt(x), T, C, _p(ws), _p(_f32vec(sub, "sub")), _p(out), _stream())
    _lib.check(rc, "ape_hip_vl_pool")
    return out


def segment_softmax(scores, nseg, gmax, out_dtype):
    _dev(scores, gmax)
    _rowmajor(scores, "scores")
    if scores.dtype != torch.float32 or gmax.dtype != torch.float32 or scores.shape[1] % nseg:
        raise ValueError("ape_amd.ops.segment_softmax: scores must be float32 [T, nseg*L], gmax a float32 scalar")
    T, C = scores.shape
    out = torch.empty((T, C), dtype=out_dtype, device=scores.device)
    rc = _lib.load().ape_hip_segment_softmax(_p(scores), _ld(scores), T, nseg, C // nseg, _p(gmax), _p(out), _ld(out), _dt(out),
                                             _stream())
    _lib.check(rc, "ape_hip_segment_softmax")
    return out


def _padded(rows, cols, pad, dtype, device):
    cp = (cols + pad - 1) // pad * pad
    out = torch.empty((rows, cp), dtype=dtype, device=device)
    if cp != cols:
        out[:, cols:].zero_()
    return out


def col_softmax_t(scores, gmax, out_dtype, pad=1):
    _dev(scores, gmax)
    _rowmajor(scores, "scores")
    if scores.dtype != torch.float32 or gmax.dtype != torch.float32:
        raise ValueError("ape_amd.ops.col_softmax_t: scores must be float32, gmax a float32 scalar")
    T, C = scores.shape
    lib = _lib.load()
    ws = torch.empty((lib.ape_hip_colstats_workspace_floats(T, C),), dtype=torch.float32, device=scores.device)
    stats = torch.empty((2, C), dtype=torch.float32, device=scores.device)
    rc = lib.ape_hip_colstats(_p(scores), _ld(scores), T, C, _p(gmax), _p(ws), _p(stats[0]), _p(stats[1]), _stream())
    _lib.check(rc, "ape_hip_colstats")
    out = _padded(C, T, pad, out_dtype, scores.device)
    rc = lib.ape_hip_transpose(_p(scores), _ld(scores), _dt(scores), T, C, _p(gmax), _p(stats[0]), _p(stats[1]), _p(out), _ld(out),
                               _dt(out), _stream())
    _lib.check(rc, "ape_hip_transpose")
    return out


def transpose(x, out_dtype=None, pad=1):
    _dev(x)
    _rowmajor(x, "x")
    T, C = x.shape
    out = _padded(C, T, pad, out_dtype or x.dtype, x.device)
    rc = _lib.load().ape_hip_transpose(_p(x), _ld(x), _dt(x), T, C, None, None, None, _p(out), _ld(out), _dt(out), _stream())
    _lib.check(rc, "ape_hip_transpose")
    return out


def mask_upsample_bits(logits, h0, w0, size):
    _dev(logits)
    _rowmajor(logits, "logits")
    n = logits.shape[0]
    out = torch.empty((n, size, size), dtype=torch.uint8, device=logits.device)
    rc = _lib.load().ape_hip_mask_upsample_bits(_p(logits), _ld(logits), _dt(logits), h0, w0, size, n, _p(out), _stream())
    _lib.check(rc, "ape_hip_mask_upsample_bits")
    return out


def roi_align_bits(bits, boxes, p):
    _dev(bits, boxes)
    n, H, W = bits.shape
    out = torch.empty((n, p, p), dtype=torch.uint8, device=bits.device)
    rc = _lib.load().ape_hip_roi_align_bits(_p(_u8(bits, "bits")), H, W, _p(_boxes(boxes)), n, p, _p(out), _stream())
    _lib.check(rc, "ape_hip_roi_align_bits")
    return out


def paste_bits(masks, boxes, ho, wo, out=None):
    _dev(masks, boxes, out)
    n, P, _ = masks.shape
    if out is None:
        out = torch.empty((n, ho, wo), dtype=torch.uint8, device=masks.device)
    elif out.dtype != torch.uint8 or tuple(out.shape) != (n, ho, wo) or not out.is_contiguous():
        raise ValueError("ape_amd.ops.paste_bits: out must be a contiguous uint8 [n, ho, wo] tensor")
    rc = _lib.load().ape_hip_paste_bits(_p(_u8(masks, "masks")), P, _p(_boxes(boxes)), n, ho, wo, _p(out), _stream())
    _lib.check(rc, "ape_hip_paste_bits")
    return out


def mask_upsample_sigmoid(logits_t, h0, w0, size, crop_h, crop_w, out_dtype):
    _dev(logits_t)
    _rowmajor(logits_t, "logits_t")
    if logits_t.shape[0] != h0 * w0:
        raise ValueError("ape_amd.ops.mask_upsample_sigmoid: logits_t must be [h0*w0, n]")
    n = logits_t.shape[1]
    out = torch.empty((crop_h * crop_w, n), dtype=out_dtype, device=logits_t.device)
    rc = _lib.load().ape_hip_mask_upsample_sigmoid(_p(logits_t), _ld(logits_t), _dt(logits_t), h0, w0, size, crop_h, crop_w, n,
                                                   _p(out), _ld(out), _dt(out), _stream())
    _lib.check(rc, "ape_hip_mask_upsample_sigmoid")
    return out


_ARANGE = {}


def arange_i64(n, device):
    key = (int(n), str(device))
    if key not in _ARANGE:
        _ARANGE[key] = torch.arange(int(n), dtype=torch.int64, device=device)
    return _ARANGE[key]


def stuff_collapse(logits, nt):
    _dev(logits)
    _rowmajor(logits, "logits")
    Q, K = logits.shape
    out = torch.empty((Q, K - nt + 1), dtype=torch.float32, device=logits.device)
    _lib.check(_lib.load().ape_hip_stuff_collapse(_p(logits), _ld(logits), Q, K, int(nt), _p(out), _ld(out), _stream()), "ape_hip_stuff_collapse")
    return out


def sem_class_weights(logits, qidx, valid, temp, kp, out_dtype):
    _dev(logits, qidx, valid)
    _rowmajor(logits, "logits")
    if qidx.dtype != torch.int64 or not qidx.is_contiguous():
        raise TypeError("ape_amd.ops.sem_class_weights: qidx must be contiguous int64")
    k, K = qidx.numel(), logits.shape[1]
    A = torch.empty((K, kp), dtype=out_dtype, device=logits.device)
    v = _f32vec(valid, "valid")
    rc = _lib.load().ape_hip_sem_class_weights(_p(logits), _ld(logits), _p(qidx), _p(v), k, int(kp), K, float(temp), _p(A), _ld(A), _dt(A), _stream())
    _lib.check(rc, "ape_hip_sem_class_weights")
    return A


def pan_class_scores(logits, qidx, valid, thresh, transform, temp):
    _dev(logits, qidx, valid)
    _rowmajor(logits, "logits")
    k = qidx.numel() if qidx is not None else logits.shape[0]
    dev = logits.device
    score = torch.empty((k,), dtype=torch.float32, device=dev)
    label = torch.empty((k,), dtype=torch.int64, device=dev)
    keep = torch.empty((k,), dtype=torch.bool, device=dev)
    label32 = torch.empty((k,), dtype=torch.int32, device=dev)
    v = _f32vec(valid, "valid")
    rc = _lib.load().ape_hip_pan_class_scores(_p(logits), _ld(logits), _p(qidx), _p(v), k, logits.shape[1], float(thresh), 1 if transform else 0,
                                              float(temp), _p(score), _p(label), _p(label32), _p(keep), _stream())
    _lib.check(rc, "ape_hip_pan_class_scores")
    return score, label, keep, label32


def argmax_labels(x, class0=None, out=None):
    _dev(x, out)
    if x.dtype != torch.float32 or x.dim() != 3 or not x.is_contiguous():
        raise ValueError("ape_amd.ops.argmax_labels: x must be contiguous float32 [C, H, W]")
    C, H, W = x.shape
    if out is None:
        out = torch.empty((H, W), dtype=torch.int16, device=x.device)
    rc = _lib.load().ape_hip_argmax_labels(_p(x), H * W, C, H * W, float("nan") if class0 is None else float(class0), _p(out), _stream())
    _lib.check(rc, "ape_hip_argmax_labels")
    return out


_LABEL_BYTES = {torch.uint8: 1, torch.int16: 2, torch.int32: 4}


def label_hist_lds_bins():
    bins = _lib.load().ape_hip_label_hist_lds_bins()
    if bins < 0:
        _lib.check(bins, "ape_hip_label_hist_lds_bins")
    return bins


def label_pair_hist(a, b, na, nb, a_ignore=None, b_ignore=None, out=None, rejected=None):
    _dev(a, b, out, rejected)
    for t, name in ((a, "a"), (b, "b")):
        if t.dtype not in _LABEL_BYTES:
            raise TypeError(f"ape_amd.ops.label_pair_hist: {name} is {t.dtype}; label maps are uint8, int16 or int32")
        if not t.is_contiguous():
            raise ValueError(f"ape_amd.ops.label_pair_hist: {name} must be contiguous")
    if a.numel() != b.numel():
        raise ValueError(f"ape_amd.ops.label_pair_hist: a has {a.numel()} labels, b has {b.numel()}")
    na, nb = int(na), int(nb)
    if na < 1 or nb < 1:
        raise ValueError("ape_amd.ops.label_pair_hist: na and nb must be at least 1")
    if out is None:
        out = torch.zeros((na, nb), dtype=torch.int64, device=a.device)
    if rejected is None:
        rejected = torch.zeros((1,), dtype=torch.int64, device=a.device)
    if (out.dtype != torch.int64 or rejected.dtype != torch.int64 or tuple(out.shape) != (na, nb) or rejected.numel() != 1
            or not out.is_contiguous()):
        raise ValueError("ape_amd.ops.label_pair_hist: out / rejected must be contiguous int64 [na, nb] / [1]")
    rc = _lib.load().ape_hip_label_pair_hist(_p(a), _LABEL_BYTES[a.dtype], _p(b), _LABEL_BYTES[b.dtype], a.numel(), na, nb,
                                             -1 if a_ignore is None else int(a_ignore), -1 if b_ignore is None else int(b_ignore),
                                             _p(out), _p(rejected), _stream())
    _lib.check(rc, "ape_hip_label_pair_hist")
    return out, rejected


def bilinear_resize(x, height, width):
    _dev(x)
    if x.dtype != torch.float32 or x.dim() != 3 or x.stride(2) != 1:
        raise ValueError("ape_amd.ops.bilinear_resize: x must be float32 [C, h, w] with contiguous rows")
    C, h, w = x.shape
    out = torch.empty((C, height, width), dtype=torch.float32, device=x.device)
    rc = _lib.load().ape_hip_bilinear_resize(_p(x), x.stride(0), x.stride(1), h, w, C, _p(out), height, width, _stream())
    _lib.check(rc, "ape_hip_bilinear_resize")
    return out


def panoptic_merge(masks, scores, keep, classes, isthing, height, width, *, prob, overlap_threshold, stuff_offset=-1):
    _dev(masks, scores, keep, classes, isthing)
    if masks.dtype != torch.float32 or masks.dim() != 3 or masks.stride(2) != 1 or scores.dtype != torch.float32:
        raise ValueError("ape_amd.ops.panoptic_merge: masks must be float32 [k, h, w] with contiguous rows, scores float32")
    k, h, w = masks.shape
    dev = masks.device
    scores = scores.contiguous()
    keep8 = keep.view(torch.uint8) if keep.dtype == torch.bool and keep.is_contiguous() else keep.to(torch.uint8).contiguous()
    cls32 = classes if classes.dtype == torch.int32 and classes.is_contiguous() else classes.to(torch.int32).contiguous()
    thing8 = isthing.view(torch.uint8) if isthing.dtype == torch.bool and isthing.is_contiguous() else isthing.to(torch.uint8).contiguous()
    owner = torch.empty((height, width), dtype=torch.int16, device=dev)
    conf = torch.empty((height, width), dtype=torch.uint8, device=dev)
    areas = torch.empty((k, 3), dtype=torch.int32, device=dev)
    seg_id = torch.empty((k,), dtype=torch.int32, device=dev)
    info = torch.empty((k, 3), dtype=torch.int32, device=dev)
    count = torch.empty((1,), dtype=torch.int32, device=dev)
    out = torch.empty((height, width), dtype=torch.int32, device=dev)
    lib = _lib.load()
    _lib.check(lib.ape_hip_panoptic_pixels(_p(masks), masks.stride(0), masks.stride(1), h, w, k, _p(scores), _p(keep8), float(prob), height, width,
                                           _p(owner), _p(conf), _p(areas), _stream()), "ape_hip_panoptic_pixels")
    _lib.check(lib.ape_hip_panoptic_decide(_p(areas), _p(cls32), _p(keep8), k, _p(thing8), thing8.numel(), float(overlap_threshold), int(stuff_offset),
                                           _p(seg_id), _p(info), _p(count), _stream()), "ape_hip_panoptic_decide")
    _lib.check(lib.ape_hip_panoptic_write(_p(owner), _p(conf), _p(seg_id), height, width, _p(out), _stream()), "ape_hip_panoptic_write")
    return out, info, count


def box_refine(delta, ref, vr4, eps=1e-3):
    _dev(delta, ref, vr4)
    if ref.dtype != torch.float32 or vr4.dtype != torch.float32 or not ref.is_contiguous() or not vr4.is_contiguous():
        raise TypeError("ape_amd.ops.box_refine: ref / vr4 must be contiguous float32")
    if delta is not None:
        _rowmajor(delta, "delta")
        if delta.dtype != torch.float32 or delta.shape != ref.shape:
            raise TypeError("ape_amd.ops.box_refine: delta must be float32 [Q,4]")
    Q, L = ref.shape[0], vr4.shape[0]
    new_ref = torch.empty_like(ref) if delta is not None else ref
    ref_in = torch.empty((Q, L, 4), dtype=torch.float32, device=ref.device)
    rc = _lib.load().ape_hip_box_refine(_p(delta), _ld(delta) if delta is not None else 0, _p(ref), _p(vr4), L, Q, float(eps),
                                        _p(new_ref) if delta is not None else None, _p(ref_in), _stream())
    _lib.check(rc, "ape_hip_box_refine")
    return new_ref, ref_in


def det_records(det_boxes, det_scores, det_classes, det_query, frame):
    _dev(det_boxes, det_scores, det_classes, det_query, frame)
    k = det_scores.numel()
    for t, dt_, n in ((det_boxes, torch.float32, 4 * k), (det_scores, torch.float32, k), (det_classes, torch.int64, k),
                      (det_query, torch.int64, k), (frame, torch.float32, 8)):
        if t.dtype != dt_ or not t.is_contiguous() or t.numel() != n:
            raise ValueError("ape_amd.ops.det_records: contiguous fp32 boxes [k,4] / scores [k] / frame [8], int64 classes / query [k]")
    dev = det_boxes.device
    rec = torch.empty((k, 8), dtype=torch.float32, device=dev)
    boxes = torch.empty((k, 4), dtype=torch.float32, device=dev)
    order = torch.empty((k,), dtype=torch.int32, device=dev)
    rc = _lib.load().ape_hip_det_records(_p(det_boxes), _p(det_scores), _p(det_classes), _p(det_query), _p(frame), k, _p(rec), _p(boxes),
                                        _p(order), _stream())
    _lib.check(rc, "ape_hip_det_records")
    return rec, boxes, order


def query_init(coords_unact, topk, dim_t, out_dtype, scale=2 * math.pi):
    _dev(coords_unact, topk, dim_t)
    if coords_unact.dtype != torch.float32 or not coords_unact.is_contiguous() or coords_unact.dim() != 2 or coords_unact.shape[1] != 4:
        raise ValueError("ape_amd.ops.query_init: coords must be contiguous float32 [T,4]")
    if topk.dtype != torch.int64 or not topk.is_contiguous():
        raise ValueError("ape_amd.ops.query_init: topk must be contiguous int64")
    T, Q, P = coords_unact.shape[0], topk.numel(), dim_t.numel()
    dev = coords_unact.device
    reference = torch.empty((Q, 4), dtype=torch.float32, device=dev)
    pe = torch.empty((Q, 4 * P), dtype=out_dtype, device=dev)
    topk32 = torch.empty((Q,), dtype=torch.int32, device=dev)
    rc = _lib.load().ape_hip_query_init(_p(coords_unact), _p(topk), T, _p(_f32vec(dim_t, "dim_t")), P, float(scale), Q, _p(reference),
                                       _p(pe), 4 * P, _dt(pe), _p(topk32), _stream())
    _lib.check(rc, "ape_hip_query_init")
    return reference, pe, topk32


def query_finish(pos, pix, norm_pos, norm_pix, out_dtype):
    _dev(pos, pix)
    _rowmajor(pos, "pos"), _rowmajor(pix, "pix")
    Q, E = pix.shape
    if pos.dtype != torch.float32 or pix.dtype != torch.float32 or pos.shape != (Q, 2 * E):
        raise ValueError("ape_amd.ops.query_finish: pos [Q, 2E] / pix [Q, E] float32")
    outs = [torch.empty((Q, E), dtype=out_dtype, device=pos.device) for _ in range(3)]
    rc = _lib.load().ape_hip_query_finish(_p(pos), _ld(pos), _p(pix), _ld(pix), Q, E, _p(_f32vec(norm_pos[0], "w")), _p(_f32vec(norm_pos[1], "b")),
                                         float(norm_pos[2]), _p(_f32vec(norm_pix[0], "w")), _p(_f32vec(norm_pix[1], "b")), float(norm_pix[2]),
                                         _p(outs[0]), _p(outs[1]), _p(outs[2]), E, _dt(outs[0]), _stream())
    _lib.check(rc, "ape_hip_query_finish")
    return tuple(outs)


_SIDE_STREAMS = {}
_FORK_DEPTH = [0]


class _Joined:
    def __init__(self, result, done=None, keep=None):
        self.result, self.done, self.keep = result, done, keep

    def join(self):
        if self.done is not None:
            torch.cuda.current_stream().wait_event(self.done)
            self.done = None
        self.keep = None
        return self.result


_FORK_INLINE = [False]
_FORK_NEST = [0]


class inline_forks:

    def __enter__(self):
        self.prev = _FORK_INLINE[0]
        _FORK_INLINE[0] = True

    def __exit__(self, *exc):
        _FORK_INLINE[0] = self.prev


def fork(fn, force=False):
    if not torch.cuda.is_available() or os.environ.get("APE_NO_FORK") == "1" or (_FORK_INLINE[0] and not force):
        return _Joined(fn())
    if _FORK_NEST[0] > 0 and os.environ.get("APE_FORK_NESTED") != "1":
        return _Joined(fn())
    dev = torch.cuda.current_device()
    cur = torch.cuda.current_stream()
    pool = _SIDE_STREAMS.setdefault((dev, cur.cuda_stream), [torch.cuda.Stream(device=dev) for _ in range(8)])
    side = pool[_FORK_DEPTH[0] % len(pool)]
    _FORK_DEPTH[0] += 1
    start = torch.cuda.Event()
    start.record(cur)
    side.wait_event(start)
    with torch.cuda.stream(side):
        _FORK_NEST[0] += 1
        try:
            result = fn()
        finally:
            _FORK_NEST[0] -= 1
        done = torch.cuda.Event()
        done.record(side)
    return _Joined(result, done, keep=fn)


def resize_coeffs(in_size, out_size):
    lib = _lib.load()
    ks = lib.ape_hip_resize_coeffs(int(in_size), int(out_size), None, None, 0)
    if ks <= 0:
        _lib.check(ks, "ape_hip_resize_coeffs")
    bounds = torch.empty((out_size, 2), dtype=torch.int32)
    kk = torch.empty((out_size, ks), dtype=torch.int32)
    rc = lib.ape_hip_resize_coeffs(int(in_size), int(out_size), ctypes.c_void_p(bounds.data_ptr()), ctypes.c_void_p(kk.data_ptr()), ks)
    if rc != ks:
        _lib.check(rc if rc < 0 else -1, "ape_hip_resize_coeffs")
    return bounds, kk


class _ResizePlan:

    def __init__(self, H, W, newh, neww, device):
        self.key = (H, W, newh, neww)
        self.bh = self.kh = self.bv = self.kv = None
        self.ks_h = self.ks_v = 0
        self.tile_h, self.lds_rows = 32, 32
        if neww != W:
            b, k = resize_coeffs(W, neww)
            self.bh, self.kh, self.ks_h = b.to(device), k.to(device), k.shape[1]
        if newh != H:
            b, k = resize_coeffs(H, newh)
            th = ctypes.c_int(0)
            rows = _lib.load().ape_hip_resize_tile_rows(ctypes.c_void_p(b.data_ptr()), newh, ctypes.byref(th))
            if rows <= 0:
                _lib.check(rows if rows < 0 else -1, "ape_hip_resize_tile_rows")
            self.tile_h, self.lds_rows = th.value, rows
            self.bv, self.kv, self.ks_v = b.to(device), k.to(device), k.shape[1]


_RESIZE_PLANS = {}


def resize_bilinear_u8(src, newh, neww, *, out=None, float_chw=False, flip=False):
    _dev(src, out)
    if src.dtype != torch.uint8 or src.dim() != 3 or src.shape[2] != 3 or src.stride(2) != 1 or src.stride(1) != 3:
        raise ValueError("ape_amd.ops.resize_bilinear_u8: src must be uint8 [H, W, 3] with packed pixels")
    H, W = src.shape[:2]
    key = (H, W, newh, neww, src.device.index)
    plan = _RESIZE_PLANS.get(key)
    if plan is None:
        if len(_RESIZE_PLANS) > 256:
            _RESIZE_PLANS.clear()
        plan = _RESIZE_PLANS[key] = _ResizePlan(H, W, newh, neww, src.device)
    if float_chw:
        if out is None:
            out = torch.empty((3, newh, neww), dtype=torch.float32, device=src.device)
        if out.dtype != torch.float32 or tuple(out.shape) != (3, newh, neww) or out.stride(2) != 1:
            raise ValueError("ape_amd.ops.resize_bilinear_u8: out must be float32 [3, newh, neww] with contiguous rows")
        kind, ld, plane = 1, out.stride(1), out.stride(0)
    else:
        if out is None:
            out = torch.empty((newh, neww, 3), dtype=torch.uint8, device=src.device)
        if out.dtype != torch.uint8 or tuple(out.shape) != (newh, neww, 3) or out.stride(2) != 1 or out.stride(1) != 3:
            raise ValueError("ape_amd.ops.resize_bilinear_u8: out must be uint8 [newh, neww, 3] with packed pixels")
        kind, ld, plane = 0, out.stride(0), 0
    rc = _lib.load().ape_hip_resize_bilinear_u8(_p(src), H, W, src.stride(0), _p(plan.bh), _p(plan.kh), plan.ks_h, _p(plan.bv),
                                                _p(plan.kv), plan.ks_v, newh, neww, plan.tile_h, plan.lds_rows, _p(out), kind,
                                                ld, plane, int(bool(flip)), _stream())
    _lib.check(rc, "ape_hip_resize_bilinear_u8")
    return out


def rle_encode(masks, cap=4096, counts=None, nruns=None):
    _dev(masks)
    if masks.dtype == torch.bool:
        masks = masks.view(torch.uint8)
    if masks.dtype != torch.uint8 or masks.dim() != 3 or not masks.is_contiguous():
        raise ValueError("ape_amd.ops.rle_encode: masks must be contiguous uint8 / bool [n, H, W]")
    n, H, W = masks.shape
    if counts is None:
        counts = torch.empty((n, cap), dtype=torch.int32, device=masks.device)
    if nruns is None:
        nruns = torch.zeros((n,), dtype=torch.int32, device=masks.device)
    _dev(counts, nruns)
    if (counts.dtype != torch.int32 or nruns.dtype != torch.int32 or tuple(counts.shape) != (n, cap) or tuple(nruns.shape) != (n,)
            or not counts.is_contiguous() or not nruns.is_contiguous()):
        raise ValueError("ape_amd.ops.rle_encode: counts / nruns must be contiguous int32 [n, cap] / [n]")
    if n == 0:
        return counts, nruns
    lib = _lib.load()
    words = lib.ape_hip_rle_workspace_words(n, H, W, cap)
    if words <= 0:
        raise ValueError("ape_amd.ops.rle_encode: workspace exceeds 2^31 words; encode fewer masks per call")
    ws = torch.empty((words,), dtype=torch.int32, device=masks.device)
    rc = lib.ape_hip_rle_encode(_p(masks), n, H, W, _p(ws), _p(counts), cap, _p(nruns), _stream())
    _lib.check(rc, "ape_hip_rle_encode")
    return counts, nruns


def rle_to_string(counts):
    c = torch.as_tensor(counts, dtype=torch.int64).to(torch.int32).contiguous() if not isinstance(counts, torch.Tensor) \
        else counts.contiguous()
    if c.is_cuda or c.dtype not in (torch.int32,):
        raise ValueError("ape_amd.ops.rle_to_string: counts must be a host int32 tensor")
    n = c.numel()
    buf = ctypes.create_string_buffer(max(8, 7 * n))
    rc = _lib.load().ape_hip_rle_to_string(ctypes.c_void_p(c.data_ptr()), n, buf, len(buf))
    if rc < 0:
        raise RuntimeError("ape_hip_rle_to_string: buffer too small")
    return buf.raw[:rc]


def rle_from_string(s):
    if isinstance(s, str):
        s = s.encode("ascii")
    if not isinstance(s, (bytes, bytearray)):
        raise TypeError(f"ape_amd.ops.rle_from_string: counts string must be bytes or str, got {type(s).__name__}")
    s = bytes(s)
    out = torch.empty((max(1, len(s)),), dtype=torch.int32)
    rc = _lib.load().ape_hip_rle_from_string(s, len(s), ctypes.c_void_p(out.data_ptr()), out.numel())
    if rc < 0:
        raise RuntimeError("ape_hip_rle_from_string: buffer too small")
    return out[:rc].clone()


def rle_decode(counts, nruns, H, W, out=None):
    _dev(counts, nruns, out)
    if counts.dtype != torch.int32 or nruns.dtype != torch.int32:
        raise TypeError(f"ape_amd.ops.rle_decode: counts / nruns must be int32, got {counts.dtype} / {nruns.dtype}")
    if counts.dim() != 2 or not counts.is_contiguous() or not nruns.is_contiguous() or tuple(nruns.shape) != (counts.shape[0],):
        raise ValueError("ape_amd.ops.rle_decode: counts / nruns must be contiguous [n, cap] / [n]")
    n, cap = counts.shape
    H, W = int(H), int(W)
    if H < 1 or W < 1 or (n > 0 and cap < 1):
        raise ValueError(f"ape_amd.ops.rle_decode: H = {H}, W = {W}, cap = {cap} must all be at least 1")
    if out is None:
        out = torch.empty((n, H, W), dtype=torch.uint8, device=counts.device)
    if out.dtype != torch.uint8 or tuple(out.shape) != (n, H, W) or not out.is_contiguous():
        raise ValueError(f"ape_amd.ops.rle_decode: out must be contiguous uint8 [{n}, {H}, {W}]")
    if n == 0:
        return out
    lib = _lib.load()
    words = lib.ape_hip_rle_decode_workspace_words(n, cap)
    if words < 0:
        raise ValueError("ape_amd.ops.rle_decode: workspace exceeds 2^31 words; decode fewer masks per call")
    ws = torch.empty((words,), dtype=torch.int32, device=counts.device)
    rc = lib.ape_hip_rle_decode(_p(counts), _p(nruns), n, cap, H, W, _p(ws), _p(out), _stream())
    _lib.check(rc, "ape_hip_rle_decode")
    return out


def _byte_masks(masks, who):
    if masks.dtype == torch.bool:
        masks = masks.view(torch.uint8)
    if masks.dtype != torch.uint8:
        raise TypeError(f"ape_amd.ops.{who}: masks are uint8 or bool, got {masks.dtype}")
    if masks.dim() != 3 or not masks.is_contiguous():
        raise ValueError(f"ape_amd.ops.{who}: masks must be contiguous [n, H, W], got shape {tuple(masks.shape)} stride {masks.stride()}")
    return masks


def mask_pack_bits(masks):
    _dev(masks)
    masks = _byte_masks(masks, "mask_pack_bits")
    n, H, W = masks.shape
    npix = H * W
    words = (npix + 63) // 64
    bits = torch.empty((n, words), dtype=torch.int64, device=masks.device)
    area = torch.empty((n,), dtype=torch.int64, device=masks.device)
    rc = _lib.load().ape_hip_mask_pack_bits(_p(masks), n, npix, npix, _p(bits), words, _p(area), _stream())
    _lib.check(rc, "ape_hip_mask_pack_bits")
    return bits, area


def mask_paired_counts(a, b, out=None):
    _dev(a, b, out)
    a, b = _byte_masks(a, "mask_paired_counts"), _byte_masks(b, "mask_paired_counts")
    if tuple(a.shape[1:]) != tuple(b.shape[1:]):
        raise ValueError(f"ape_amd.ops.mask_paired_counts: masks of {tuple(a.shape[1:])} against masks of {tuple(b.shape[1:])}")
    if a.shape[0] != b.shape[0]:
        raise ValueError(f"ape_amd.ops.mask_paired_counts: {a.shape[0]} masks against {b.shape[0]}; the counts are of pairs (a_i, b_i)")
    if a.device != b.device or (out is not None and out.device != a.device):
        raise ValueError("ape_amd.ops.mask_paired_counts: a, b and out must be on one device")
    n, H, W = a.shape
    npix = H * W
    if out is None:
        out = torch.empty((n, 3), dtype=torch.int64, device=a.device)
    if out.dtype != torch.int64 or tuple(out.shape) != (n, 3) or not out.is_contiguous():
        raise ValueError(f"ape_amd.ops.mask_paired_counts: out must be contiguous int64 [{n}, 3]")
    if n == 0:
        return out
    rc = _lib.load().ape_hip_mask_paired_counts(_p(a), npix, _p(b), npix, n, npix, _p(out), _stream())
    _lib.check(rc, "ape_hip_mask_paired_counts")
    return out


def bitmask_pair_counts(a_bits, b_bits, out=None):
    _dev(a_bits, b_bits, out)
    for t, name in ((a_bits, "a_bits"), (b_bits, "b_bits")):
        if t.dtype != torch.int64:
            raise TypeError(f"ape_amd.ops.bitmask_pair_counts: {name} is {t.dtype}; packed masks are int64 words")
        if t.dim() != 2 or not t.is_contiguous():
            raise ValueError(f"ape_amd.ops.bitmask_pair_counts: {name} must be contiguous [rows, words]")
    if a_bits.shape[1] != b_bits.shape[1]:
        raise ValueError(f"ape_amd.ops.bitmask_pair_counts: a_bits has {a_bits.shape[1]} words per mask, b_bits has {b_bits.shape[1]}")
    n, m, words = a_bits.shape[0], b_bits.shape[0], a_bits.shape[1]
    if out is None:
# ... 397 lines not shown
```

ape_amd/packing.py:

```python
import torch


def round_up(x, m):
    return (x + m - 1) // m * m


def pack_matrix(w, dtype, kpad=8, rows=None):
    N, K = w.shape
    Kp = round_up(K, kpad)
    Np = rows or N
    out = torch.zeros((Np, Kp), dtype=dtype, device=w.device)
    out[:N, :K] = w.detach().to(dtype)
    return out


def ffn_w2_perm(hid):
    assert hid % 32 == 0
    pos = torch.arange(hid)
    grp, r = pos // 32, pos % 32
    g, e = r // 8, r % 8
    return grp * 32 + torch.where(e < 4, 4 * g + e, 16 + 4 * g + (e - 4))


def permute_ffn_w2(w2):
    return w2[:, ffn_w2_perm(w2.shape[1]).to(w2.device)].contiguous()


def f32(t):
    return None if t is None else t.detach().float().contiguous()


def ln_params(norm):
    return f32(norm.weight), f32(norm.bias), norm.eps


class PackCache:

    def __init__(self):
        self._store = {}

    def get(self, module, dtype, builder):
        p = next(module.parameters(), None)
        key = (dtype, p.device if p is not None else None)
        if key not in self._store:
            with torch.no_grad():
                self._store[key] = builder(dtype)
        return self._store[key]

    def clear(self):
        self._store.clear()


def attach_cache(module):
    module._pack = PackCache()
    module.register_load_state_dict_post_hook(lambda m, incompatible: m._pack.clear())


def _cubic_axis_weights(n_in, n_out):
    import math

    import numpy as np
    A = -0.75

    def near(x):
        return ((A + 2.0) * x - (A + 3.0)) * x * x + 1.0

    def far(x):
        return ((A * x - 5.0 * A) * x + 8.0 * A) * x - 4.0 * A
    W = np.zeros((n_out, n_in), dtype=np.float64)
    scale = n_in / n_out
    for o in range(n_out):
        src = scale * (o + 0.5) - 0.5
        i0 = math.floor(src)
        t = src - i0
        for k, wk in enumerate((far(t + 1.0), near(t), near(1.0 - t), far(2.0 - t))):
            W[o, min(max(i0 - 1 + k, 0), n_in - 1)] += wk
    return W


def resize_pos_embed(pos, size, hw):
    import numpy as np

    from . import ops
    w1 = _cubic_axis_weights(size, hw)
    kron = torch.from_numpy(np.kron(w1, w1).astype(np.float32)).to(pos.device)
    return ops.gemm(kron, pos.detach().float().t().contiguous(), None, out_dtype=torch.float32)
```

include/ape_hip.h:

```cpp
#ifndef APE_HIP_H
#define APE_HIP_H
#include <stdint.h>

#ifdef __cplusplus
extern "C" {
#endif

#define APE_DT_F32 0
#define APE_DT_BF16 1
#define APE_DT_F16 2

#define APE_ACT_NONE 0
#define APE_ACT_RELU 1
#define APE_ACT_GELU 2
#define APE_ACT_SWIGLU 3
#define APE_ACT_SILU 4

#define APE_MASK_NONE 0
#define APE_MASK_ZERO_INPUT 1
#define APE_MASK_ZERO_OUTPUT 2

const char* ape_hip_last_error(void);
int ape_hip_abi_version(void);
int ape_hip_sizeof_args(int which);

typedef struct ApeGemmArgs {
  const void* A;
  const void* W;
  void* C;
  const float* bias;
  const void* residual;
  const uint8_t* rowmask;
  const float* rope_cos;
  const float* rope_sin;
  int32_t M, N, K;
  int32_t lda, ldw, ldc, ldr;
  int32_t in_dt, out_dt, res_dt;
  int32_t act;
  int32_t mask_mode;
  int32_t trans_out;
  int32_t rope_rows, rope_hd, rope_cols;
  int32_t vec_ok;
  float alpha;
  float clamp;
  int32_t splitk;
  int32_t tile64;
  float* workspace;
  const float* rowscale;
  const float* rowshift;
  const float* colvec;
  const float* rope_cs;
  const float* ln_w;
  const float* ln_b;
  float ln_eps;
  int32_t reserved0;
  const int32_t* conv_perm;
  const void* conv_zero;
  int32_t conv_h, conv_w;
  int32_t rowstat_cols;
  float rowstat_eps;
} ApeGemmArgs;
int ape_hip_gemm(const ApeGemmArgs* args, void* stream);
const char* ape_hip_gemm_last_kernel(void);

int ape_hip_meter_begin(void);
int ape_hip_meter_count(void);
int ape_hip_meter_end(void);
int ape_hip_meter_read(int i, const char** name, float* ms);
int ape_hip_zero(void* ptr, size_t nbytes, void* stream);
int ape_hip_sdma_usable(const void* host_dst, const void* dev_src);
int ape_hip_sdma_d2h(void* host_dst, const void* dev_src, size_t nbytes);
int ape_hip_sdma_d2h_multi(int n, void* const* host_dst, const void* const* dev_src, const size_t* nbytes, int parts);
int ape_hip_sdma_engines(const void* host_dst, const void* dev_src);

int ape_hip_row_stats(const void* x, int ldx, int dt, int M, int C, float eps, float* rowscale, float* rowshift, void* stream);

int ape_hip_gemv(const float* x, int ldx, const void* W, int ldw, int w_dt, const float* bias, float* out, int ldo,
                 int M, int N, int K, float alpha, void* stream);
int ape_hip_gemv_affine(const float* x, int ldx, const void* W, int ldw, int w_dt, const float* bias, float* out, int ldo,
                        int M, int N, int K, float alpha, const float* scale, const float* add, int ldadd, float* out2, int ldo2,
                        void* stream);

typedef struct ApeLayerNormArgs {
  const void* x;
  const float* w;
  const float* b;
  void* y;
  const void* add;
  void* y2;
  int32_t M, C, Cpad;
  int32_t ldx, ldy, ldadd, ldy2;
  int32_t x_dt, y_dt, add_dt;
  int32_t act;
  float eps;
} ApeLayerNormArgs;
int ape_hip_layernorm(const ApeLayerNormArgs* args, void* stream);

int ape_hip_postnorm_residual(const void* t, int ldt, int t_dt, const float* w, const float* b, float eps, float* stream, int lds,
                              void* copy, int ldc, int copy_dt, int M, int C, void* hip_stream);


typedef struct ApeGroupNormArgs {
  const void* x;
  const float* w;
  const float* b;
  void* y;
  const void* add;
  float* workspace;
  int32_t HW, C, G;
  int32_t ldx, ldy, ldadd;
  int32_t x_dt, y_dt, add_dt;
  int32_t act;
  float eps;
} ApeGroupNormArgs;
int ape_hip_groupnorm_workspace_floats(int HW, int G);
int ape_hip_groupnorm(const ApeGroupNormArgs* args, void* stream);

int ape_hip_ms_deform_attn_forward(const void* value, int ldv, const int64_t* spatial_shapes,
                                   const int64_t* level_start_index, const void* sampling_loc,
                                   const void* attn_weight, void* out, int ldout, int B, int S, int Q, int L,
                                   int dt, void* stream);
int ape_hip_msda_fused(const void* value, int ldv, int v_dt, const int64_t* spatial_shapes,
                       const int64_t* level_start_index, const float* offw, int ldoffw, const float* ref,
                       int refdim, void* out, int ldout, int out_dt, int B, int S, int Q, int L, void* stream);
int ape_hip_msda_fused_h(const void* value, int ldv, int v_dt, const int64_t* spatial_shapes,
                       const int64_t* level_start_index, const void* offw_f16, int ldoffw, const float* ref,
                       int refdim, void* out, int ldout, int out_dt, int B, int S, int Q, int L, void* stream);

int ape_hip_attention(const void* Q, int ldq, const void* K, int ldk, const void* Vt, int ldvt, void* O, int ldo,
                      int B, int N, int H, int HD, float scale, int dt, void* stream);
int ape_hip_attention_strided(const void* Q, int ldq, const void* K, int ldk, const void* Vt, int ldvt, void* O, int ldo,
                              int B, int N, int bstride, int H, int HD, float scale, int dt, void* stream);
int ape_hip_attention_causal(const void* Q, int ldq, const void* K, int ldk, const void* Vt, int ldvt, void* O, int ldo,
                              int B, int N, int bstride, int H, int HD, float scale, int dt, void* stream);


int ape_hip_patchify(const float* img, int h, int w, const int32_t* tok2raster, int Ht, int Wt, const float* mean3,
                     const float* std3, void* out, int ldo, int out_dt, void* stream);
int ape_hip_im2col3x3(const void* x, int ldx, const int32_t* perm, int H, int W, int C, void* out, int ldo, int dt, void* stream);
int ape_hip_maxpool2x2(const void* x, int ldx, const int32_t* perm, int H, int W, int C, void* out, int ldo, int dt, void* stream);
int ape_hip_gather_rows(const void* x, int ldx, const int32_t* idx, int n, int C, void* out, int ldo, int dt, void* stream);
int ape_hip_gather_rows_i64(const void* x, int ldx, const int64_t* idx, int n, int C, void* out, int ldo, int dt, void* stream);

int ape_hip_nms_mask_words(int n);
int ape_hip_nms_mask(const float* boxes_xyxy, const int32_t* groups, int n, float iou_thr, uint64_t* mask, void* stream);
int ape_hip_nms_scan_segments(const uint64_t* mask, int n, const int32_t* seg_offsets, int num_segments, int max_segment,
                              const uint8_t* valid, uint8_t* keep, void* stream);
int ape_hip_nms_scan_classes(const uint64_t* mask, int n, const int32_t* order, int num_classes, const uint8_t* valid,
                             uint8_t* keep, void* stream);

int ape_hip_vl_pool_workspace_floats(int T, int C);
int ape_hip_vl_pool(const float* S, int lds, const void* x, int ldx, int x_dt, int T, int C, float* workspace, const float* sub,
                    float* out, void* stream);
int ape_hip_head_gemv(const float* x, int ldx, const float* W, const float* bias, float* out, int ldo, int H, int N, int D,
                      float alpha, void* out_bf16, int ldob, int copy_dt, void* stream);

int ape_hip_segment_softmax(const float* S, int lds, int T, int nseg, int L, const float* gmax, void* out, int ldo, int out_dt,
                            void* stream);
int ape_hip_colstats_workspace_floats(int T, int C);
int ape_hip_colstats(const float* S, int lds, int T, int C, const float* gmax, float* workspace, float* colmax, float* colsum,
                     void* stream);
int ape_hip_transpose(const void* S, int lds, int in_dt, int T, int C, const float* gmax, const float* colmax,
                      const float* colsum, void* out, int ldo, int out_dt, void* stream);
int ape_hip_stuff_collapse(const float* logits, int ldl, int Q, int K, int nt, float* out, int ldo, void* stream);
int ape_hip_sem_class_weights(const float* logits, int ldl, const int64_t* qidx, const float* valid_score, int k, int kp, int K, float temp,
                              void* A, int lda, int out_dt, void* stream);
int ape_hip_pan_class_scores(const float* logits, int ldl, const int64_t* qidx, const float* valid_score, int k, int K, float thresh, int transform,
                             float temp, float* score, int64_t* label, int32_t* label32 , uint8_t* keep, void* stream);
int ape_hip_argmax_labels(const float* x, size_t ld_class, int C, size_t n, float class0, int16_t* out, void* stream);


int ape_hip_mask_upsample_bits(const void* logits, int ldl, int dt, int h0, int w0, int S, int n, uint8_t* out, void* stream);
int ape_hip_roi_align_bits(const uint8_t* bits, int H, int W, const float* boxes, int n, int P, uint8_t* out, void* stream);
int ape_hip_paste_bits(const uint8_t* masks, int P, const float* boxes, int n, int Ho, int Wo, uint8_t* out, void* stream);

int ape_hip_mask_upsample_sigmoid(const void* logits, int ldl, int in_dt, int h0, int w0, int S, int crop_h, int crop_w, int n,
                                  void* out, int ldo, int out_dt, void* stream);
int ape_hip_bilinear_resize(const float* in, int ld_channel, int ld_row, int h, int w, int C, float* out, int H, int W,
                            void* stream);

int ape_hip_panoptic_pixels(const float* masks, int ld_query, int ld_row, int h, int w, int k, const float* scores, const uint8_t* keep,
                            float prob, int H, int W, int16_t* owner, uint8_t* conf, int* areas, void* stream);
int ape_hip_panoptic_decide(const int* areas, const int* classes, const uint8_t* keep, int k, const uint8_t* isthing, int num_classes,
                            double overlap_threshold, int stuff_offset, int* seg_id, int* info, int* count, void* stream);
int ape_hip_panoptic_write(const int16_t* owner, const uint8_t* conf, const int* seg_id, int H, int W, int* out, void* stream);

int ape_hip_box_refine(const float* delta, int ldd, const float* ref, const float* vr4, int L, int Q, float eps, float* new_ref,
                       float* ref_in, void* stream);

int ape_hip_det_records(const float* boxes, const float* scores, const int64_t* classes, const int64_t* query, const float* frame,
                        int k, float* rec, float* boxes_out, int32_t* order, void* stream);
int ape_hip_query_init(const float* coords, const int64_t* topk, int T, const float* dim_t, int P, float scale, int Q,
                       float* reference, void* pe, int ldpe, int pe_dt, int32_t* topk32, void* stream);
int ape_hip_query_finish(const float* pos, int ldpos, const float* pix, int ldpix, int Q, int E, const float* wpos,
                         const float* bpos, float eps_pos, const float* wpix, const float* bpix, float eps_pix, void* query_pos,
                         void* query, void* query_sum, int ldo, int out_dt, void* stream);

int ape_hip_geometry(int S, int h, int w, int L, const int* level_hw, const float* dim_t, int npf, const float* level_embeds,
                     float offset, float eps, float scale, void* lvl_pos, int lvl_pos_dt, uint8_t* mask_u8, uint8_t* mask_bool,
                     uint8_t* invalid_u8, float* enc_ref, float* proposals, float* valid_ratios, float* vr4, float* box_scale,
                     void* stream);

int ape_hip_resize_coeffs(int in_size, int out_size, int32_t* bounds, int32_t* kk, int ksize_cap);
int ape_hip_resize_tile_rows(const int32_t* bounds_v_host, int newh, int* tile_h);
int ape_hip_resize_bilinear_u8(const uint8_t* src, int H, int W, int src_ld, const int32_t* bounds_h, const int32_t* kk_h,
                               int ks_h, const int32_t* bounds_v, const int32_t* kk_v, int ks_v, int newh, int neww, int tile_h,
                               int lds_rows, void* dst, int dst_kind, int dst_ld, int dst_plane, int flip, void* stream);

int ape_hip_rle_workspace_words(int n, int H, int W, int cap);
int ape_hip_rle_encode(const uint8_t* masks, int n, int H, int W, uint32_t* workspace, uint32_t* counts, int cap, uint32_t* nruns,
                       void* stream);
int ape_hip_rle_to_string(const uint32_t* counts, int n, char* out, int cap);

int ape_hip_embed_tokens(const int32_t* tokens, int ldt, const void* table, int ldtab, const void* pos, int ldpos, int dt, float* out,
                         int ldo, int B, int L, int Lp, int W, int vocab, void* stream);

int ape_hip_enc_finalize(const float* cls2, const float* d, const float* anchors, int T, float* enc_class, float* enc_coord,
                         float* xyxy, void* stream);
int ape_hip_topk_workspace_words(int n_total);
int ape_hip_proposal_topk(const float* logit, int T, const int* level_start, const int* level_n, int L, int k, int k_alt,
                          uint64_t* workspace, int32_t* cand, int32_t* alt, void* stream);
int ape_hip_proposal_order(const int32_t* cand, int n, const float* logit, const float* xyxy, const int* level_start,
                           const int* level_n, int L, float* boxes_b, int32_t* groups_b, int32_t* seg, int32_t* cand_a,
                           int32_t* lv_a, int32_t* pos_b, void* stream);
int ape_hip_proposal_quota(const int32_t* cand_a, const int32_t* lv_a, const int32_t* pos_b, const uint8_t* keep_b, int n,
                           const int32_t* alt, int n_alt, const int* level_start, const int* level_n, int L, int nq, int64_t* out,
                           void* stream);
int ape_hip_det_sort(const float* logits, int ldl, int Q, int K, const float* boxes, const float* scale, float thresh, float* xyxy,
                     uint8_t* finite, float* sorted, int32_t* order, uint8_t* valid, void* stream);
int ape_hip_det_topk(const float* sorted, const uint8_t* keep, const int32_t* order, const float* xyxy, int K, int Q, int k,
                     uint64_t* workspace, float* det_boxes, float* det_scores, int64_t* det_classes, int64_t* det_query, void* stream);

int ape_hip_attention_ext(const void* Q, int ldq, const void* K, int ldk, const void* Vt, int ldvt, void* O, int ldo, int B, int N,
                          int bstride, int H, int HDQ, int HDV, float scale, int dt, void* stream);
int ape_hip_relpos_extend(const void* q, const void* k, int ldqk, const void* t, int ldt, int tper, const int* ty, const int* tx, int period,
                          void* q_ext, void* k_ext, int lde, int rows, int nh, int hs, int hd, int Hk, int Wk, int hdq, float scale, int dt,
                          void* stream);

int ape_hip_ffn_fused(const void* X, int ldx, const void* W1, int ldw1, const float* b1, const void* W2, int ldw2, const float* b2,
                      const void* residual, int ldr, void* Y, int ldy, int M, int K, int HID, int N, int w2_permuted, int dt,
                      const float* ln_weight, const float* ln_bias, float ln_eps, void* stream);

int ape_hip_label_hist_lds_bins(void);
int ape_hip_label_pair_hist(const void* a, int a_bytes, const void* b, int b_bytes, size_t n, int na, int nb, int a_ignore,
                            int b_ignore, int64_t* hist, int64_t* rejected, void* stream);

int ape_hip_mask_pack_bits(const uint8_t* masks, int n, size_t npix, size_t stride, uint64_t* bits, size_t ldb, int64_t* area,
                           void* stream);
int ape_hip_mask_paired_counts(const uint8_t* a, size_t stride_a, const uint8_t* b, size_t stride_b, int n, size_t npix, int64_t* out,
                               void* stream);
int ape_hip_bitmask_pair_counts(const uint64_t* a, int n, size_t lda, const uint64_t* b, int m, size_t ldb, size_t words,
                                int64_t* inter, size_t ldi, void* stream);
int ape_hip_rle_decode_workspace_words(int n, int cap);
int ape_hip_rle_decode(const uint32_t* counts, const uint32_t* nruns, int n, int cap, int H, int W, uint32_t* workspace,
                       uint8_t* masks, void* stream);
int ape_hip_rle_from_string(const char* s, int len, uint32_t* counts, int cap);

int ape_hip_mask_pack_rows(const uint8_t* masks, int n, int H, int W, uint64_t* bits, size_t ldb, int64_t* area, void* stream);
int ape_hip_bitmask_boundary(const uint64_t* bits, int n, int H, int W, int d, size_t ldb, uint64_t* bbits, size_t ldo, int64_t* barea,
                             void* stream);
int ape_hip_bitmask_boundary_tile(int H, int W, int d, size_t lds_limit, int* tile_rows, int* tile_words);
int ape_hip_bitmask_unpack_rows(const uint64_t* bits, int n, int H, int W, size_t ldb, uint8_t* masks, void* stream);

int ape_hip_box_cover_overlaps(const float* proposals, int n, const float* gt, const float* gt_area, int m, const float* ranges,
                               const int* limits, int C, float* overlaps, int* match, void* stream);

int ape_hip_coco_match(const double* iou, int n, int m, size_t ld, const int* det_order, int nd, const int* det_offsets,
                       const int* gt_order, int ng, const int* gt_offsets, int K, const uint8_t* gt_crowd, const double* gt_area,
                       const double* det_area, const double* thresholds, int T, const double* ranges, int A, int* match,
                       uint8_t* flag, void* stream);

#ifdef __cplusplus
}
#endif
#endif
```

Measured before the change: 114.6.

## Fuse deformable decoder layer tail into two chained per-row-block HIP kernels

Adds two fused kernels for the DETR-style decoder: one chains the attention output projection, residual add, layernorm, query-pos add and offset/weight projection. The other chains the output projection, LN1, the FFN (two GEMMs with ReLU), LN2 and the box MLP with reference refinement. Each block keeps 16 query rows in LDS across the stages and streams pre-packed MFMA-fragment weights. The goal is to remove many small kernel launches and intermediate global round-trips for the small query count. The cost is a larger LDS footprint, few blocks per launch (Q/16) and extra weight packing. The fused path can be switched off with an environment variable.

```diff
diff --git a/ape_amd/_lib.py b/ape_amd/_lib.py
--- a/ape_amd/_lib.py
+++ b/ape_amd/_lib.py
@@ -174,6 +174,13 @@
                                            c_void_p]),
     "ape_hip_coco_match": (c_int, [c_void_p, c_int, c_int, ctypes.c_size_t, c_void_p, c_int, c_void_p, c_void_p, c_int, c_void_p, c_int,
                                    c_void_p, c_void_p, c_void_p, c_void_p, c_int, c_void_p, c_int, c_void_p, c_void_p, c_void_p]),
+    "ape_hip_dec_chain_c": (c_int, [c_void_p, c_int, c_void_p, c_int, c_void_p, c_int, c_int, c_int, c_void_p, c_void_p, c_void_p, c_void_p,
+                                    c_float, c_void_p, c_void_p, c_int, c_void_p, c_int, c_void_p, c_int, c_void_p, c_void_p, c_int,
+                                    c_void_p, c_void_p]),
+    "ape_hip_dec_chain_t": (c_int, [c_void_p, c_int, c_void_p, c_int, c_void_p, c_int, c_int, c_int, c_void_p, c_void_p, c_void_p, c_void_p,
+                                    c_float, c_void_p, c_void_p, c_void_p, c_void_p, c_int, c_int, c_void_p, c_void_p, c_float, c_void_p,
+                                    c_void_p, c_void_p, c_void_p, c_void_p, c_void_p, c_void_p, c_void_p, c_int, c_float, c_void_p, c_int,
+                                    c_void_p, c_int, c_void_p, c_void_p, c_void_p, c_void_p]),
 }
 
 _lib = None
diff --git a/ape_amd/csrc/boxes.hip b/ape_amd/csrc/boxes.hip
--- a/ape_amd/csrc/boxes.hip
+++ b/ape_amd/csrc/boxes.hip
@@ -1,5 +1,6 @@
 #include "common.h"
 #include "../../include/ape_hip.h"
+#include "row_ops.h"
 
 __global__ __launch_bounds__(256) void box_refine_kernel(const float* __restrict__ delta, int ldd, const float* __restrict__ ref,
                                                          const float* __restrict__ vr4, int L, int Q, float eps,
@@ -7,12 +8,7 @@
   const int gid = blockIdx.x * 256 + threadIdx.x;
   if (gid >= Q * 4) return;
   const int q = gid >> 2, c = gid & 3;
-  float x = ref[gid];
-  x = fminf(fmaxf(x, 0.f), 1.f);
-  const float x1 = fmaxf(x, eps), x2 = fmaxf(1.f - x, eps);
-  float z = logf(x1 / x2);
-  if (delta != nullptr) z += delta[(size_t)q * ldd + c];
-  const float r = delta != nullptr ? 1.f / (1.f + expf(-z)) : ref[gid];
+  const float r = box_refine_value(ref[gid], delta != nullptr, delta != nullptr ? delta[(size_t)q * ldd + c] : 0.f, eps);
   if (new_ref != nullptr) new_ref[gid] = r;
   if (ref_in != nullptr)
     for (int l = 0; l < L; ++l) ref_in[((size_t)q * L + l) * 4 + c] = r * vr4[l * 4 + c];
@@ -199,3 +195,5 @@
   APE_CHECK_LAUNCH("ape_hip_det_records");
   return 0;
 }
+
+#include "dec_chain.h"
diff --git a/ape_amd/csrc/dec_chain.h b/ape_amd/csrc/dec_chain.h
--- /dev/null
+++ b/ape_amd/csrc/dec_chain.h
@@ -0,0 +1,368 @@
+#pragma once
+#include "common.h"
+#include "../../include/ape_hip.h"
+
+#include "gemm_epi.h"
+#include "row_ops.h"
+
+#define DC_ROWS 16
+#define DC_E 256
+#define DC_P (DC_E + 8)
+#define DC_WAVES 8
+#define DC_THREADS (DC_WAVES * 64)
+#define DC_DEPTH 4
+#define DC_MAX_HIDDEN 2048
+#define DC_MAX_OFFW 512
+
+template <typename H> __device__ __forceinline__ bf16x8_t dc_frag(const H* p) {
+  return __builtin_bit_cast(bf16x8_t, *reinterpret_cast<const short8_t*>(p));
+}
+
+template <typename H>
+__device__ __forceinline__ void dc_load_block(H* dst, const H* __restrict__ src, int ld, int row0, int M, int tid) {
+  for (int c = tid; c < DC_ROWS * (DC_E / 8); c += DC_THREADS) {
+    const int r = c >> 5, k = c & 31;
+    int gr = row0 + r; gr = gr < M ? gr : M - 1;
+    *reinterpret_cast<uint4*>(dst + r * DC_P + k * 8) = *reinterpret_cast<const uint4*>(src + (size_t)gr * ld + k * 8);
+  }
+}
+template <typename H>
+__device__ __forceinline__ void dc_store_block(H* __restrict__ dst, int ld, const H* src, int row0, int M, int tid) {
+  for (int c = tid; c < DC_ROWS * (DC_E / 8); c += DC_THREADS) {
+    const int r = c >> 5, k = c & 31;
+    if (row0 + r < M) *reinterpret_cast<uint4*>(dst + (size_t)(row0 + r) * ld + k * 8) = *reinterpret_cast<const uint4*>(src + r * DC_P + k * 8);
+  }
+}
+__device__ __forceinline__ void dc_load_f32(float* dst, const float* __restrict__ src, int n, int tid) {
+  for (int i = tid * 4; i < n; i += DC_THREADS * 4) *reinterpret_cast<float4*>(dst + i) = *reinterpret_cast<const float4*>(src + i);
+}
+
+__device__ __forceinline__ GemmParams dc_epi(int N, const float* bias, int act, const void* residual, int ldr, int res_dt) {
+  GemmParams p = {};
+  p.M = DC_ROWS; p.N = N;
+  p.bias = bias; p.act = act;
+  p.residual = residual; p.ldr = ldr; p.res_dt = res_dt;
+  p.mask_mode = APE_MASK_NONE;
+  p.alpha = 1.f; p.clamp = 0.f;
+  p.vec_ok = 1 | 2;
+  return p;
+}
+
+template <typename H, bool KE, int D, typename Sink>
+__device__ __forceinline__ void dc_gemm(const H* sA, int lda, const H* __restrict__ W, int N, int K, int nparts, const GemmParams& ep,
+                                        int lane, int wave, Sink&& sink) {
+  const int frow = lane & 15, fq = lane >> 4;
+  const int tiles = (N + 15) >> 4;
+  const int mytiles = tiles > wave ? (tiles - wave + DC_WAVES - 1) / DC_WAVES : 0;
+  if (mytiles == 0) return;
+  const int KC = KE ? 1 : (K >> 8);
+  const int nsteps = mytiles * KC;
+  const int per_split = (K >> 5) / nparts;
+  bf16x8_t areg[8];
+  if (KE) {
+#pragma unroll
+    for (int j = 0; j < 8; ++j) areg[j] = dc_frag<H>(sA + frow * lda + j * 32 + fq * 8);
+  }
+  bf16x8_t wb[D][8];
+  int it = 0, ikc = 0;
+  auto issue = [&](bf16x8_t (&dst)[8]) {
+    const int t = wave + DC_WAVES * (it < mytiles ? it : mytiles - 1);
+    const H* src = W + (((size_t)t * (K >> 5) + ikc * 8) * 64 + lane) * 8;
+#pragma unroll
+    for (int j = 0; j < 8; ++j) dst[j] = dc_frag<H>(src + j * 512);
+    if (++ikc == KC) { ikc = 0; ++it; }
+  };
+  int ct = 0, ckc = 0, ktd = 0;
+  f32x4_t acc = {0.f, 0.f, 0.f, 0.f}, sum = {0.f, 0.f, 0.f, 0.f};
+  auto consume = [&](bf16x8_t (&src)[8]) {
+#pragma unroll
+    for (int j = 0; j < 8; ++j) {
+      const bf16x8_t af = KE ? areg[j] : dc_frag<H>(sA + frow * lda + ckc * 256 + j * 32 + fq * 8);
+      acc = h16<H>::mfma(src[j], af, acc);
+    }
+    ktd += 8;
+    if (nparts > 1 && ktd == per_split) {
+#pragma unroll
+      for (int r = 0; r < 4; ++r) sum[r] += acc[r];
+      acc = (f32x4_t){0.f, 0.f, 0.f, 0.f};
+      ktd = 0;
+    }
+    if (++ckc == KC) {
+      const int n0 = (wave + DC_WAVES * ct) * 16 + fq * 4;
+      if (ct < mytiles && n0 < N) {
+        float v[4];
+#pragma unroll
+        for (int r = 0; r < 4; ++r) v[r] = nparts > 1 ? sum[r] : acc[r];
+        int ocol, cnt;
+        epi_n4_values<H>(ep, frow, n0, v, ocol, cnt);
+        sink(frow, ocol, v);
+      }
+      acc = (f32x4_t){0.f, 0.f, 0.f, 0.f};
+      sum = (f32x4_t){0.f, 0.f, 0.f, 0.f};
+      ckc = 0; ktd = 0; ++ct;
+    }
+  };
+#pragma unroll
+  for (int d = 0; d < D; ++d) issue(wb[d]);
+  int s0 = 0;
+  for (; s0 + D < nsteps; s0 += D) {
+#pragma unroll
+    for (int d = 0; d < D; ++d) { consume(wb[d]); issue(wb[d]); }
+  }
+#pragma unroll
+  for (int d = 0; d < D; ++d) consume(wb[d]);
+}
+
+template <typename H>
+__device__ __forceinline__ void dc_sink_h(H* dst, int pitch, int row, int col, const float* v) {
+  *reinterpret_cast<uint2*>(dst + row * pitch + col) = make_uint2(h16<H>::pack2(v[0], v[1]), h16<H>::pack2(v[2], v[3]));
+}
+
+template <typename H>
+__device__ __forceinline__ void dc_ln(const H* sx, H* sy, const H* sadd, H* sy2, const float* w, const float* b, float eps, int wave, int lane) {
+  for (int r = wave; r < DC_ROWS; r += DC_WAVES)
+    ln_row<H, H, H, 1>(sx + r * DC_P, sy + r * DC_P, sadd != nullptr ? sadd + r * DC_P : nullptr, sy2 != nullptr ? sy2 + r * DC_P : nullptr, w, b,
+                       DC_E, DC_E, eps, APE_ACT_NONE, lane);
+}
+
+__device__ __forceinline__ void dc_ref_in(float r, int q, int c, const float* __restrict__ vr4, int L, float* __restrict__ ref_in) {
+  for (int l = 0; l < L; ++l) ref_in[((size_t)q * L + l) * 4 + c] = r * vr4[l * 4 + c];
+}
+
+struct DecChainC {
+  const void *o, *x, *qpos, *wo, *woffw;
+  const float *bo, *ln_w, *ln_b, *boffw, *ref, *vr4;
+  void* x2;
+  float *offw, *ref_in;
+  int ldo, ldx, ldq, ldx2, ldoffw, M, noffw, L;
+  float eps;
+};
+#define DC_C_PAR (3 * DC_E + DC_MAX_OFFW)
+#define DC_C_LDS (DC_C_PAR * 4 + 6 * DC_ROWS * DC_P * 2)
+
+template <typename H>
+__global__ __launch_bounds__(DC_THREADS) void dec_chain_c_kernel(const DecChainC a) {
+  extern __shared__ __attribute__((aligned(16))) unsigned char dc_smem[];
+  float* sBo = reinterpret_cast<float*>(dc_smem);
+  float* sLw = sBo + DC_E;
+  float* sLb = sLw + DC_E;
+  float* sBoff = sLb + DC_E;
+  H* sO = reinterpret_cast<H*>(sBoff + DC_MAX_OFFW);
+  H* sX = sO + DC_ROWS * DC_P;
+  H* sQ = sX + DC_ROWS * DC_P;
+  H* sX1 = sQ + DC_ROWS * DC_P;
+  H* sX2 = sX1 + DC_ROWS * DC_P;
+  H* sX2p = sX2 + DC_ROWS * DC_P;
+  const int tid = threadIdx.x, lane = tid & 63, wave = tid >> 6;
+  const int row0 = blockIdx.x * DC_ROWS;
+  const int M = a.M;
+  dc_load_f32(sBo, a.bo, DC_E, tid);
+  dc_load_f32(sLw, a.ln_w, DC_E, tid);
+  dc_load_f32(sLb, a.ln_b, DC_E, tid);
+  dc_load_f32(sBoff, a.boffw, a.noffw, tid);
+  dc_load_block<H>(sO, reinterpret_cast<const H*>(a.o), a.ldo, row0, M, tid);
+  dc_load_block<H>(sX, reinterpret_cast<const H*>(a.x), a.ldx, row0, M, tid);
+  dc_load_block<H>(sQ, reinterpret_cast<const H*>(a.qpos), a.ldq, row0, M, tid);
+  __syncthreads();
+  {
+    const GemmParams ep = dc_epi(DC_E, sBo, APE_ACT_NONE, sX, DC_P, h16<H>::dt);
+    dc_gemm<H, true, 2>(sO, DC_P, reinterpret_cast<const H*>(a.wo), DC_E, DC_E, 1, ep, lane, wave,
+                     [&](int r, int c, const float* v) { dc_sink_h<H>(sX1, DC_P, r, c, v); });
+  }
+  __syncthreads();
+  dc_ln<H>(sX1, sX2, sQ, sX2p, sLw, sLb, a.eps, wave, lane);
+  __syncthreads();
+  dc_store_block<H>(reinterpret_cast<H*>(a.x2), a.ldx2, sX2, row0, M, tid);
+  {
+    const GemmParams ep = dc_epi(a.noffw, sBoff, APE_ACT_NONE, nullptr, 0, APE_DT_F32);
+    float* offw = a.offw;
+    const int ldoffw = a.ldoffw;
+    dc_gemm<H, true, DC_DEPTH>(sX2p, DC_P, reinterpret_cast<const H*>(a.woffw), a.noffw, DC_E, 1, ep, lane, wave, [&](int r, int c, const float* v) {
+      if (row0 + r < M) *reinterpret_cast<float4*>(offw + (size_t)(row0 + r) * ldoffw + c) = make_float4(v[0], v[1], v[2], v[3]);
+    });
+  }
+  if (a.ref_in != nullptr && tid < 64) {
+    const int q = row0 + (tid >> 2), c = tid & 3;
+    if (q < M) dc_ref_in(box_refine_value(a.ref[q * 4 + c], false, 0.f, 0.f), q, c, a.vr4, a.L, a.ref_in);
+  }
+}
+
+struct DecChainT {
+  const void *samp, *x2, *qpos, *wout, *w1, *w2, *wb1, *wb2, *wb3;
+  const float *bout, *ln1_w, *ln1_b, *b1, *b2, *ln2_w, *ln2_b, *bb1, *bb2, *bb3, *ref, *vr4;
+  void *out, *outp;
+  float *delta, *new_ref, *ref_in;
+  int lds, ldx2, ldq, ldout, ldoutp, M, hidden, splitk, L;
+  float eps1, eps2, box_eps;
+};
+#define DC_T_PAR (9 * DC_E + DC_MAX_HIDDEN + 16 + DC_ROWS * 4)
+static inline int dc_t_lds(int hidden) { return DC_T_PAR * 4 + 7 * DC_ROWS * DC_P * 2 + DC_ROWS * (hidden + 8) * 2; }
+
+template <typename H>
+__global__ __launch_bounds__(DC_THREADS) void dec_chain_t_kernel(const DecChainT a) {
+  extern __shared__ __attribute__((aligned(16))) unsigned char dc_smem[];
+  float* sBout = reinterpret_cast<float*>(dc_smem);
+  float* sL1w = sBout + DC_E;
+  float* sL1b = sL1w + DC_E;
+  float* sB2 = sL1b + DC_E;
+  float* sL2w = sB2 + DC_E;
+  float* sL2b = sL2w + DC_E;
+  float* sBb1 = sL2b + DC_E;
+  float* sBb2 = sBb1 + DC_E;
+  float* sB1 = sBb2 + DC_E;
+  float* sBb3 = sB1 + DC_MAX_HIDDEN;
+  float* sDelta = sBb3 + 16;
+  H* sSamp = reinterpret_cast<H*>(sDelta + DC_ROWS * 4);
+  H* sX2 = sSamp + DC_ROWS * DC_P;
+  H* sQ = sX2 + DC_ROWS * DC_P;
+  H* sX3 = sQ + DC_ROWS * DC_P;
+  H* sX4 = sX3 + DC_ROWS * DC_P;
+  H* sOut = sX4 + DC_ROWS * DC_P;
+  H* sOutp = sOut + DC_ROWS * DC_P;
+  H* sHid = sOutp + DC_ROWS * DC_P;
+  const int tid = threadIdx.x, lane = tid & 63, wave = tid >> 6;
+  const int row0 = blockIdx.x * DC_ROWS;
+  const int M = a.M, hidden = a.hidden, hp = hidden + 8;
+  const bool box = a.wb1 != nullptr;
+  dc_load_f32(sBout, a.bout, DC_E, tid);
+  dc_load_f32(sL1w, a.ln1_w, DC_E, tid);
+  dc_load_f32(sL1b, a.ln1_b, DC_E, tid);
+  dc_load_f32(sB2, a.b2, DC_E, tid);
+  dc_load_f32(sL2w, a.ln2_w, DC_E, tid);
+  dc_load_f32(sL2b, a.ln2_b, DC_E, tid);
+  dc_load_f32(sB1, a.b1, hidden, tid);
+  if (box) {
+    dc_load_f32(sBb1, a.bb1, DC_E, tid);
+    dc_load_f32(sBb2, a.bb2, DC_E, tid);
+    dc_load_f32(sBb3, a.bb3, 4, tid);
+  }
+  dc_load_block<H>(sSamp, reinterpret_cast<const H*>(a.samp), a.lds, row0, M, tid);
+  dc_load_block<H>(sX2, reinterpret_cast<const H*>(a.x2), a.ldx2, row0, M, tid);
+  dc_load_block<H>(sQ, reinterpret_cast<const H*>(a.qpos), a.ldq, row0, M, tid);
+  __syncthreads();
+  {
+    const GemmParams ep = dc_epi(DC_E, sBout, APE_ACT_NONE, sX2, DC_P, h16<H>::dt);
+    dc_gemm<H, true, 2>(sSamp, DC_P, reinterpret_cast<const H*>(a.wout), DC_E, DC_E, 1, ep, lane, wave,
+                     [&](int r, int c, const float* v) { dc_sink_h<H>(sX3, DC_P, r, c, v); });
+  }
+  __syncthreads();
+  dc_ln<H>(sX3, sX4, nullptr, nullptr, sL1w, sL1b, a.eps1, wave, lane);
+  __syncthreads();
+  {
+    const GemmParams ep = dc_epi(hidden, sB1, APE_ACT_RELU, nullptr, 0, APE_DT_F32);
+    dc_gemm<H, true, DC_DEPTH>(sX4, DC_P, reinterpret_cast<const H*>(a.w1), hidden, DC_E, 1, ep, lane, wave,
+                     [&](int r, int c, const float* v) { dc_sink_h<H>(sHid, hp, r, c, v); });
+  }
+  __syncthreads();
+  {
+    const GemmParams ep = dc_epi(DC_E, sB2, APE_ACT_NONE, sX4, DC_P, h16<H>::dt);
+    dc_gemm<H, false, DC_DEPTH>(sHid, hp, reinterpret_cast<const H*>(a.w2), DC_E, hidden, a.splitk, ep, lane, wave,
+                      [&](int r, int c, const float* v) { dc_sink_h<H>(sSamp, DC_P, r, c, v); });
+  }
+  __syncthreads();
+  dc_ln<H>(sSamp, sOut, sQ, sOutp, sL2w, sL2b, a.eps2, wave, lane);
+  __syncthreads();
+  dc_store_block<H>(reinterpret_cast<H*>(a.out), a.ldout, sOut, row0, M, tid);
+  dc_store_block<H>(reinterpret_cast<H*>(a.outp), a.ldoutp, sOutp, row0, M, tid);
+  if (!box) return;
+  {
+    const GemmParams ep = dc_epi(DC_E, sBb1, APE_ACT_RELU, nullptr, 0, APE_DT_F32);
+    dc_gemm<H, true, 2>(sOut, DC_P, reinterpret_cast<const H*>(a.wb1), DC_E, DC_E, 1, ep, lane, wave,
+                     [&](int r, int c, const float* v) { dc_sink_h<H>(sX3, DC_P, r, c, v); });
+  }
+  __syncthreads();
+  {
+    const GemmParams ep = dc_epi(DC_E, sBb2, APE_ACT_RELU, nullptr, 0, APE_DT_F32);
+    dc_gemm<H, true, 2>(sX3, DC_P, reinterpret_cast<const H*>(a.wb2), DC_E, DC_E, 1, ep, lane, wave,
+                     [&](int r, int c, const float* v) { dc_sink_h<H>(sX2, DC_P, r, c, v); });
+  }
+  __syncthreads();
+  {
+    const GemmParams ep = dc_epi(4, sBb3, APE_ACT_NONE, nullptr, 0, APE_DT_F32);
+    float* delta = a.delta;
+    dc_gemm<H, true, 1>(sX2, DC_P, reinterpret_cast<const H*>(a.wb3), 4, DC_E, 1, ep, lane, wave, [&](int r, int c, const float* v) {
+      *reinterpret_cast<float4*>(sDelta + r * 4) = make_float4(v[0], v[1], v[2], v[3]);
+      if (row0 + r < M) *reinterpret_cast<float4*>(delta + (size_t)(row0 + r) * 4) = make_float4(v[0], v[1], v[2], v[3]);
+    });
+  }
+  __syncthreads();
+  if (tid < 64) {
+    const int q = row0 + (tid >> 2), c = tid & 3;
+    if (q < M) {
+      const float r = box_refine_value(a.ref[q * 4 + c], true, sDelta[tid], a.box_eps);
+      a.new_ref[q * 4 + c] = r;
+      dc_ref_in(r, q, c, a.vr4, a.L, a.ref_in);
+    }
+  }
+}
+
+static bool dc_al16(const void* p) { return p != nullptr && ((uintptr_t)p) % 16 == 0; }
+
+extern "C" int ape_hip_dec_chain_c(const void* o, int ldo, const void* x, int ldx, const void* qpos, int ldq, int Q, int dt, const void* wo,
+                                   const float* bo, const float* ln_w, const float* ln_b, float eps, const void* woffw, const float* boffw,
+                                   int noffw, void* x2, int ldx2, float* offw, int ldoffw, const float* ref, const float* vr4, int L,
+                                   float* ref_in, void* stream) {
+  APE_CHECK_ARG(ape_is16(dt), "ape_hip_dec_chain_c: 16-bit storage (bf16 | f16) only; fp32 runs the separate launches");
+  APE_CHECK_ARG(Q > 0 && noffw > 0 && noffw % 16 == 0 && noffw <= DC_MAX_OFFW && ldoffw >= noffw && ldoffw % 4 == 0,
+                "ape_hip_dec_chain_c: Q > 0, offset width a multiple of 16 up to %d, ldoffw %% 4 == 0", DC_MAX_OFFW);
+  APE_CHECK_ARG(dc_al16(o) && dc_al16(x) && dc_al16(qpos) && dc_al16(wo) && dc_al16(woffw) && dc_al16(bo) && dc_al16(ln_w) && dc_al16(ln_b) &&
+                    dc_al16(boffw) && dc_al16(x2) && dc_al16(offw),
+                "ape_hip_dec_chain_c: null or unaligned pointer (16 bytes)");
+  APE_CHECK_ARG(ldo >= DC_E && ldx >= DC_E && ldq >= DC_E && ldx2 >= DC_E && ldo % 8 == 0 && ldx % 8 == 0 && ldq % 8 == 0 && ldx2 % 8 == 0,
+                "ape_hip_dec_chain_c: rows of 256 16-bit values, 16-byte aligned");
+  APE_CHECK_ARG(ref_in == nullptr || (ref != nullptr && vr4 != nullptr && L > 0), "ape_hip_dec_chain_c: ref_in needs ref, vr4 and L > 0");
+  DecChainC a;
+  a.o = o; a.x = x; a.qpos = qpos; a.wo = wo; a.woffw = woffw;
+  a.bo = bo; a.ln_w = ln_w; a.ln_b = ln_b; a.boffw = boffw; a.ref = ref; a.vr4 = vr4;
+  a.x2 = x2; a.offw = offw; a.ref_in = ref_in;
+  a.ldo = ldo; a.ldx = ldx; a.ldq = ldq; a.ldx2 = ldx2; a.ldoffw = ldoffw; a.M = Q; a.noffw = noffw; a.L = L;
+  a.eps = eps;
+  const dim3 grid(ceil_div(Q, DC_ROWS)), block(DC_THREADS);
+  hipStream_t s = (hipStream_t)stream;
+  if (dt == APE_DT_F16) APE_LAUNCH(dec_chain_c_kernel<f16_t>, grid, block, DC_C_LDS, s, a);
+  else APE_LAUNCH(dec_chain_c_kernel<bf16_t>, grid, block, DC_C_LDS, s, a);
+  APE_CHECK_LAUNCH("ape_hip_dec_chain_c");
+  return 0;
+}
+
+extern "C" int ape_hip_dec_chain_t(const void* samp, int lds, const void* x2, int ldx2, const void* qpos, int ldq, int Q, int dt,
+                                   const void* wout, const float* bout, const float* ln1_w, const float* ln1_b, float eps1, const void* w1,
+                                   const float* b1, const void* w2, const float* b2, int hidden, int splitk, const float* ln2_w,
+                                   const float* ln2_b, float eps2, const void* wb1, const float* bb1, const void* wb2, const float* bb2,
+                                   const void* wb3, const float* bb3, const float* ref, const float* vr4, int L, float box_eps, void* out,
+                                   int ldout, void* outp, int ldoutp, float* delta, float* new_ref, float* ref_in, void* stream) {
+  APE_CHECK_ARG(ape_is16(dt), "ape_hip_dec_chain_t: 16-bit storage (bf16 | f16) only; fp32 runs the separate launches");
+  APE_CHECK_ARG(Q > 0 && hidden >= 256 && hidden % 256 == 0 && hidden <= DC_MAX_HIDDEN, "ape_hip_dec_chain_t: hidden width a multiple of 256 up to %d",
+                DC_MAX_HIDDEN);
+  APE_CHECK_ARG(splitk >= 1 && (hidden / 32) % splitk == 0 && (splitk == 1 || (hidden / 32 / splitk) % 8 == 0),
+                "ape_hip_dec_chain_t: K partitions of a multiple of 256 columns (hidden %d, splitk %d)", hidden, splitk);
+  APE_CHECK_ARG(dc_al16(samp) && dc_al16(x2) && dc_al16(qpos) && dc_al16(wout) && dc_al16(w1) && dc_al16(w2) && dc_al16(bout) && dc_al16(ln1_w) &&
+                    dc_al16(ln1_b) && dc_al16(b1) && dc_al16(b2) && dc_al16(ln2_w) && dc_al16(ln2_b) && dc_al16(out) && dc_al16(outp),
+                "ape_hip_dec_chain_t: null or unaligned pointer (16 bytes)");
+  APE_CHECK_ARG(lds >= DC_E && ldx2 >= DC_E && ldq >= DC_E && ldout >= DC_E && ldoutp >= DC_E && lds % 8 == 0 && ldx2 % 8 == 0 && ldq % 8 == 0 &&
+                    ldout % 8 == 0 && ldoutp % 8 == 0,
+                "ape_hip_dec_chain_t: rows of 256 16-bit values, 16-byte aligned");
+  if (wb1 != nullptr) {
+    APE_CHECK_ARG(dc_al16(wb1) && dc_al16(wb2) && dc_al16(wb3) && dc_al16(bb1) && dc_al16(bb2) && dc_al16(bb3) && dc_al16(delta) && dc_al16(new_ref) &&
+                      dc_al16(ref_in) && ref != nullptr && vr4 != nullptr && L > 0,
+                  "ape_hip_dec_chain_t: the box head needs its three layers, delta / new_ref / ref_in (16-byte aligned), ref, vr4 and L > 0");
+  }
+  DecChainT a;
+  a.samp = samp; a.x2 = x2; a.qpos = qpos; a.wout = wout; a.w1 = w1; a.w2 = w2; a.wb1 = wb1; a.wb2 = wb2; a.wb3 = wb3;
+  a.bout = bout; a.ln1_w = ln1_w; a.ln1_b = ln1_b; a.b1 = b1; a.b2 = b2; a.ln2_w = ln2_w; a.ln2_b = ln2_b; a.bb1 = bb1; a.bb2 = bb2; a.bb3 = bb3;
+  a.ref = ref; a.vr4 = vr4;
+  a.out = out; a.outp = outp; a.delta = delta; a.new_ref = new_ref; a.ref_in = ref_in;
+  a.lds = lds; a.ldx2 = ldx2; a.ldq = ldq; a.ldout = ldout; a.ldoutp = ldoutp; a.M = Q; a.hidden = hidden; a.splitk = splitk; a.L = L;
+  a.eps1 = eps1; a.eps2 = eps2; a.box_eps = box_eps;
+  static ApeOncePerDevice attr_done;
+  if (attr_done.first()) {
+    (void)hipFuncSetAttribute((const void*)dec_chain_t_kernel<bf16_t>, hipFuncAttributeMaxDynamicSharedMemorySize, dc_t_lds(DC_MAX_HIDDEN));
+    (void)hipFuncSetAttribute((const void*)dec_chain_t_kernel<f16_t>, hipFuncAttributeMaxDynamicSharedMemorySize, dc_t_lds(DC_MAX_HIDDEN));
+  }
+  const dim3 grid(ceil_div(Q, DC_ROWS)), block(DC_THREADS);
+  hipStream_t s = (hipStream_t)stream;
+  if (dt == APE_DT_F16) APE_LAUNCH(dec_chain_t_kernel<f16_t>, grid, block, dc_t_lds(hidden), s, a);
+  else APE_LAUNCH(dec_chain_t_kernel<bf16_t>, grid, block, dc_t_lds(hidden), s, a);
+  APE_CHECK_LAUNCH("ape_hip_dec_chain_t");
+  return 0;
+}
diff --git a/ape_amd/csrc/norm.hip b/ape_amd/csrc/norm.hip
--- a/ape_amd/csrc/norm.hip
+++ b/ape_amd/csrc/norm.hip
@@ -1,11 +1,6 @@
 #include "common.h"
 #include "../../include/ape_hip.h"
-
-__device__ __forceinline__ float ln_act(float x, int act) {
-  if (act == APE_ACT_RELU) return fmaxf(x, 0.f);
-  if (act == APE_ACT_GELU) return 0.5f * x * (1.f + erff(x * 0.70710678118654752440f));
-  return x;
-}
+#include "row_ops.h"
 
 template <typename TX, typename TY, typename TA, int NV4>
 __global__ __launch_bounds__(256) void layernorm_kernel(const ApeLayerNormArgs p) {
@@ -16,70 +11,7 @@
   TY* y = reinterpret_cast<TY*>(p.y) + (size_t)row * p.ldy;
   const TA* add = p.add ? reinterpret_cast<const TA*>(p.add) + (size_t)row * p.ldadd : nullptr;
   TY* y2 = p.y2 ? reinterpret_cast<TY*>(p.y2) + (size_t)row * p.ldy2 : nullptr;
-  const int C = p.C;
-  const float invC = 1.f / (float)C;
-  float v[NV4][4];
-  float s = 0.f;
-#pragma unroll
-  for (int i = 0; i < NV4; ++i) {
-    const int c = (i * 64 + lane) * 4;
-    if (c + 3 < C) {
-      ld4<TX>(x + c, v[i]);
-    } else {
-#pragma unroll
-      for (int r = 0; r < 4; ++r) v[i][r] = (c + r < C) ? ldf<TX>(x + c + r) : 0.f;
-    }
-    s += (v[i][0] + v[i][1]) + (v[i][2] + v[i][3]);
-  }
-  const float mean = wave_sum(s) * invC;
-  float q = 0.f;
-#pragma unroll
-  for (int i = 0; i < NV4; ++i) {
-    const int c = (i * 64 + lane) * 4;
-#pragma unroll
-    for (int r = 0; r < 4; ++r) {
-      const float d = (c + r < C) ? v[i][r] - mean : 0.f;
-      q = fmaf(d, d, q);
-    }
-  }
-  const float rstd = rsqrtf(wave_sum(q) * invC + p.eps);
-#pragma unroll
-  for (int i = 0; i < NV4; ++i) {
-    const int c = (i * 64 + lane) * 4;
-    if (c >= p.Cpad) continue;
-    float o[4], o2[4];
-    if (c + 3 < C) {
-      float w4[4], b4[4];
-      ld4<float>(p.w + c, w4);
-      ld4<float>(p.b + c, b4);
-#pragma unroll
-      for (int r = 0; r < 4; ++r) o[r] = ln_act((v[i][r] - mean) * rstd * w4[r] + b4[r], p.act);
-      st4<TY>(y + c, o);
-      if (y2 != nullptr) {
-        ld4<TA>(add + c, o2);
-#pragma unroll
-        for (int r = 0; r < 4; ++r) o2[r] += o[r];
-        st4<TY>(y2 + c, o2);
-      }
-      continue;
-    }
-#pragma unroll
-    for (int r = 0; r < 4; ++r) {
-      if (c + r < C) {
-        o[r] = ln_act((v[i][r] - mean) * rstd * p.w[c + r] + p.b[c + r], p.act);
-        o2[r] = (y2 != nullptr) ? o[r] + ldf<TA>(add + c + r) : 0.f;
-      } else {
-        o[r] = 0.f; o2[r] = 0.f;
-      }
-    }
-    if (c + 3 < p.Cpad) {
-      st4<TY>(y + c, o);
-      if (y2 != nullptr) st4<TY>(y2 + c, o2);
-    } else {
-      for (int r = 0; r < 4 && c + r < p.Cpad; ++r) { stf<TY>(y + c + r, o[r]); if (y2 != nullptr) stf<TY>(y2 + c + r, o2[r]); }
-    }
-  }
-  for (int c = NV4 * 256 + lane; c < p.Cpad; c += 64) { stf<TY>(y + c, 0.f); if (y2 != nullptr) stf<TY>(y2 + c, 0.f); }
+  ln_row<TX, TY, TA, NV4>(x, y, add, y2, p.w, p.b, p.C, p.Cpad, p.eps, p.act, lane);
 }
 
 template <typename TX, typename TY, typename TA>
diff --git a/ape_amd/csrc/row_ops.h b/ape_amd/csrc/row_ops.h
--- /dev/null
+++ b/ape_amd/csrc/row_ops.h
@@ -0,0 +1,86 @@
+#pragma once
+#include "common.h"
+#include "../../include/ape_hip.h"
+
+__device__ __forceinline__ float ln_act(float x, int act) {
+  if (act == APE_ACT_RELU) return fmaxf(x, 0.f);
+  if (act == APE_ACT_GELU) return 0.5f * x * (1.f + erff(x * 0.70710678118654752440f));
+  return x;
+}
+
+template <typename TX, typename TY, typename TA, int NV4>
+__device__ __forceinline__ void ln_row(const TX* x, TY* y, const TA* add, TY* y2, const float* w, const float* b, int C, int Cpad,
+                                       float eps, int act, int lane) {
+  const float invC = 1.f / (float)C;
+  float v[NV4][4];
+  float s = 0.f;
+#pragma unroll
+  for (int i = 0; i < NV4; ++i) {
+    const int c = (i * 64 + lane) * 4;
+    if (c + 3 < C) {
+      ld4<TX>(x + c, v[i]);
+    } else {
+#pragma unroll
+      for (int r = 0; r < 4; ++r) v[i][r] = (c + r < C) ? ldf<TX>(x + c + r) : 0.f;
+    }
+    s += (v[i][0] + v[i][1]) + (v[i][2] + v[i][3]);
+  }
+  const float mean = wave_sum(s) * invC;
+  float q = 0.f;
+#pragma unroll
+  for (int i = 0; i < NV4; ++i) {
+    const int c = (i * 64 + lane) * 4;
+#pragma unroll
+    for (int r = 0; r < 4; ++r) {
+      const float d = (c + r < C) ? v[i][r] - mean : 0.f;
+      q = fmaf(d, d, q);
+    }
+  }
+  const float rstd = rsqrtf(wave_sum(q) * invC + eps);
+#pragma unroll
+  for (int i = 0; i < NV4; ++i) {
+    const int c = (i * 64 + lane) * 4;
+    if (c >= Cpad) continue;
+    float o[4], o2[4];
+    if (c + 3 < C) {
+      float w4[4], b4[4];
+      ld4<float>(w + c, w4);
+      ld4<float>(b + c, b4);
+#pragma unroll
+      for (int r = 0; r < 4; ++r) o[r] = ln_act((v[i][r] - mean) * rstd * w4[r] + b4[r], act);
+      st4<TY>(y + c, o);
+      if (y2 != nullptr) {
+        ld4<TA>(add + c, o2);
+#pragma unroll
+        for (int r = 0; r < 4; ++r) o2[r] += o[r];
+        st4<TY>(y2 + c, o2);
+      }
+      continue;
+    }
+#pragma unroll
+    for (int r = 0; r < 4; ++r) {
+      if (c + r < C) {
+        o[r] = ln_act((v[i][r] - mean) * rstd * w[c + r] + b[c + r], act);
+        o2[r] = (y2 != nullptr) ? o[r] + ldf<TA>(add + c + r) : 0.f;
+      } else {
+        o[r] = 0.f; o2[r] = 0.f;
+      }
+    }
+    if (c + 3 < Cpad) {
+      st4<TY>(y + c, o);
+      if (y2 != nullptr) st4<TY>(y2 + c, o2);
+    } else {
+      for (int r = 0; r < 4 && c + r < Cpad; ++r) { stf<TY>(y + c + r, o[r]); if (y2 != nullptr) stf<TY>(y2 + c + r, o2[r]); }
+    }
+  }
+  for (int c = NV4 * 256 + lane; c < Cpad; c += 64) { stf<TY>(y + c, 0.f); if (y2 != nullptr) stf<TY>(y2 + c, 0.f); }
+}
+
+__device__ __forceinline__ float box_refine_value(float ref, bool has_delta, float delta, float eps) {
+  float x = ref;
+  x = fminf(fmaxf(x, 0.f), 1.f);
+  const float x1 = fmaxf(x, eps), x2 = fmaxf(1.f - x, eps);
+  float z = logf(x1 / x2);
+  if (has_delta) z += delta;
+  return has_delta ? 1.f / (1.f + expf(-z)) : ref;
+}
diff --git a/ape_amd/layers/multi_scale_deform_attn.py b/ape_amd/layers/multi_scale_deform_attn.py
--- a/ape_amd/layers/multi_scale_deform_attn.py
+++ b/ape_amd/layers/multi_scale_deform_attn.py
@@ -84,12 +84,15 @@
             value = ops.gemm(value_src, P["wval"], P["bval"], rowmask=mask, mask_mode=ops.MASK_ZERO_OUTPUT,
                              **half_value_kwargs(dt, value_src.shape[0]))
         half = dt in ops.HALF16 and query_pos_sum.shape[0] >= 2048 and os.environ.get("APE_MSDA_F32_OFFSETS") != "1"
-        offw = ops.gemm(query_pos_sum, P["woffw"], P["boffw"], out_dtype=torch.float16 if half else torch.float32)[:, :P["noffw"]]
-        samp = ops.msda_fused(value, shapes, starts, offw, ref, out_dtype=dt)
+        offw = ops.gemm(query_pos_sum, P["woffw"], P["boffw"], out_dtype=torch.float16 if half else torch.float32)
+        samp = self.sample_tokens(offw, value, ref, shapes, starts, dt)
         if norm is not None and ops.gemm_norm_fusable(samp, P["wout"], identity, out_dtype):
             return ops.gemm(samp, P["wout"], P["bout"], residual=identity, norm=norm)
         y = ops.gemm(samp, P["wout"], P["bout"], residual=identity, out_dtype=out_dtype or dt)
         return y if norm is None else ops.layernorm(y, norm[0], norm[1], norm[2], out_dtype=out_dtype or dt)
+
+    def sample_tokens(self, offw, value, ref, shapes, starts, dt):
+        return ops.msda_fused(value, shapes, starts, offw[:, :self.packed(dt)["noffw"]], ref, out_dtype=dt)
 
     def forward(self, query, key=None, value=None, identity=None, query_pos=None, key_padding_mask=None,
                 reference_points=None, spatial_shapes=None, level_start_index=None, **kwargs):
diff --git a/ape_amd/modeling/ape_deta/_containers.py b/ape_amd/modeling/ape_deta/_containers.py
--- a/ape_amd/modeling/ape_deta/_containers.py
+++ b/ape_amd/modeling/ape_deta/_containers.py
@@ -82,15 +82,18 @@
                         wo=pack_matrix(self.attn.out_proj.weight, dt), bo=f32(self.attn.out_proj.bias))
         return self._pack.get(self, dt, build)
 
-    def forward_tokens(self, x, x_pos, dt, vt_buf, out_dtype=None):
+    def attend_tokens(self, x, x_pos, dt, vt_buf):
         P = self.packed(dt)
         E, nh = self.embed_dim, self.num_heads
         hd = E // nh
         vjob = ops.fork(lambda: ops.gemm(x, P["wv"], P["bv"], trans_out=True, out=vt_buf))
         qk = ops.gemm(x_pos, P["wqk"], P["bqk"])
         vt = vjob.join()
-        o = ops.attention(qk[:, :E], qk[:, E:], vt, batch=1, n=x.shape[0], heads=nh, head_dim=hd, scale=hd ** -0.5)
-        return ops.gemm(o, P["wo"], P["bo"], residual=x, out_dtype=out_dtype or dt)
+        return ops.attention(qk[:, :E], qk[:, E:], vt, batch=1, n=x.shape[0], heads=nh, head_dim=hd, scale=hd ** -0.5)
+
+    def forward_tokens(self, x, x_pos, dt, vt_buf, out_dtype=None):
+        P = self.packed(dt)
+        return ops.gemm(self.attend_tokens(x, x_pos, dt, vt_buf), P["wo"], P["bo"], residual=x, out_dtype=out_dtype or dt)
 
 
 class TransformerLayer(nn.Module):
diff --git a/ape_amd/modeling/ape_deta/deformable_transformer_vl.py b/ape_amd/modeling/ape_deta/deformable_transformer_vl.py
--- a/ape_amd/modeling/ape_deta/deformable_transformer_vl.py
+++ b/ape_amd/modeling/ape_deta/deformable_transformer_vl.py
@@ -5,7 +5,7 @@
 
 from ... import ops
 from ...layers import MultiScaleDeformableAttention
-from ...packing import attach_cache, f32, ln_params, pack_matrix, round_up
+from ...packing import attach_cache, f32, ln_params, pack_fragments, pack_matrix, round_up
 from ...stagetap import forcing, tap
 from . import geometry as G
 from ._containers import FFN, SelfAttention, TransformerLayer
@@ -74,7 +74,16 @@
         def build(dt):
             ws = [l.attentions[1].value_proj.weight for l in self.layers]
             bs = [l.attentions[1].value_proj.bias.detach().float() for l in self.layers]
-            return dict(wval=pack_matrix(torch.cat(ws, 0), dt), bval=torch.cat(bs).contiguous())
+            P = dict(wval=pack_matrix(torch.cat(ws, 0), dt), bval=torch.cat(bs).contiguous())
+            if dt in ops.HALF16:
+                P["chains"] = []
+                for i, l in enumerate(self.layers):
+                    Ps, Pc, Pf = l.attentions[0].packed(dt), l.attentions[1].packed(dt), l.ffns[0].packed(dt)
+                    box = self.bbox_embed[i].packed(dt) if self.bbox_embed is not None else None
+                    P["chains"].append(dict(wo=pack_fragments(Ps["wo"]), woffw=pack_fragments(Pc["woffw"]), wout=pack_fragments(Pc["wout"]),
+                                            w1=pack_fragments(Pf["w1"]), w2=pack_fragments(Pf["w2"]),
+                                            box=None if box is None else [(pack_fragments(w), b) for w, b in box]))
+            return P
         return self._pack.get(self, dt, build)
 
     def forward_tokens(self, query, query_pos, memory, geo, reference, dt, stages=None, query_sum=None):
@@ -89,6 +98,9 @@
         out = query
         outp = query_sum if query_sum is not None else (query.float() + query_pos.float()).to(dt)
         inter, inter_ref = [], []
+        hidden = self.layers[0].ffns[0].layers[1].weight.shape[1]
+        if not forcing(stages) and ops.dec_chain_fusable(out, outp, query_pos, dt=dt, hidden=hidden):
+            return self._forward_chains(out, outp, query_pos, value_all, geo, reference.contiguous(), vr4, vt_buf, dt, stages)
         _, ref_in = ops.box_refine(None, reference.contiguous(), vr4)
         refjob = ops._Joined((reference, ref_in))
         for i, layer in enumerate(self.layers):
@@ -122,6 +134,35 @@
         reference, _ = refjob.join()
         reference = tap(stages, f"dec{len(self.layers) - 1}_ref", reference)
         inter_ref.append(reference)
+        return inter, inter_ref
+
+
+    def _forward_chains(self, out, outp, query_pos, value_all, geo, reference, vr4, vt_buf, dt, stages):
+        E = self.embed_dim
+        inter, inter_ref = [], []
+        ref_in = None
+        for i, layer in enumerate(self.layers):
+            sa, ca = layer.attentions
+            Ps, Pc, Pf, F = sa.packed(dt), ca.packed(dt), layer.ffns[0].packed(dt), self.packed(dt)["chains"][i]
+            o = sa.attend_tokens(out, outp, dt, vt_buf)
+            if ref_in is None:
+                x2, offw, ref_in = ops.dec_chain_c(o, out, query_pos, F["wo"], Ps["bo"], layer.norm_params(0), F["woffw"], Pc["boffw"],
+                                                   ref=reference, vr4=vr4)
+            else:
+                x2, offw = ops.dec_chain_c(o, out, query_pos, F["wo"], Ps["bo"], layer.norm_params(0), F["woffw"], Pc["boffw"])
+            if i > 0:
+                inter_ref.append(tap(stages, f"dec{i - 1}_ref", reference))
+            samp = ca.sample_tokens(offw, value_all[:, i * E:(i + 1) * E], ref_in, geo.shapes, geo.starts, dt)
+            box = F["box"]
+            out, outp, delta, new_ref, new_ref_in = ops.dec_chain_t(samp, x2, query_pos, F["wout"], Pc["bout"], layer.norm_params(1), F["w1"],
+                                                                    Pf["b1"], F["w2"], Pf["b2"], layer.norm_params(2), box=box,
+                                                                    ref=reference, vr4=vr4)
+            tap(stages, f"dec{i}_out", out)
+            if box is not None:
+                tap(stages, f"dec{i}_delta", delta)
+                reference, ref_in = new_ref, new_ref_in
+            inter.append(out)
+        inter_ref.append(tap(stages, f"dec{len(self.layers) - 1}_ref", reference))
         return inter, inter_ref
 
 
diff --git a/ape_amd/ops.py b/ape_amd/ops.py
--- a/ape_amd/ops.py
+++ b/ape_amd/ops.py
@@ -828,6 +828,93 @@
     return new_ref, ref_in
 
 
+DEC_CHAIN = [os.environ.get("APE_NO_DEC_CHAIN") != "1"]
+DEC_CHAIN_MAX_ROWS = 2048
+
+
+def _dec_chain_splitk(rows, hidden, dtype):
+    return _auto_tiling(rows, 256, hidden, dtype, False, ACT_NONE)[1]
+
+
+def dec_chain_fusable(*rows, dt, hidden):
+    if not DEC_CHAIN[0] or dt not in HALF16 or not rows:
+        return False
+    for t in rows:
+        if not (torch.is_tensor(t) and t.is_cuda and t.dtype == dt and t.dim() == 2 and t.shape[1] == 256 and t.stride(1) == 1
+                and _ld(t) % 8 == 0 and t.data_ptr() % 16 == 0 and 0 < t.shape[0] < DEC_CHAIN_MAX_ROWS):
+            return False
+    if hidden % 256 != 0 or not 256 <= hidden <= 2048:
+        return False
+    sk = _dec_chain_splitk(rows[0].shape[0], hidden, dt)
+    return (hidden // 32) % sk == 0 and (sk == 1 or (hidden // 32 // sk) % 8 == 0)
+
+
+def _chain_rows(dt, Q, **ts):
+    for name, t in ts.items():
+        _rowmajor(t, name)
+        if t.dtype != dt or tuple(t.shape) != (Q, 256):
+            raise ValueError(f"ape_amd.ops.dec_chain: {name} must be {dt} [{Q}, 256], got {t.dtype} {tuple(t.shape)}")
+
+
+def _chain_weight(w, dt, n, k, name):
+    if w.dtype != dt or tuple(w.shape) != ((n + 15) // 16, k // 32, 64, 8) or not w.is_contiguous():
+        raise ValueError(f"ape_amd.ops.dec_chain: {name} must be packing.pack_fragments of a {dt} [{n}, {k}] matrix, got {w.dtype} {tuple(w.shape)}")
+    return w
+
+
+def dec_chain_c(o, x, qpos, wo, bo, norm, woffw, boffw, *, ref=None, vr4=None):
+    _dev(o, x, qpos, wo, bo, woffw, boffw, norm[0], norm[1], ref, vr4)
+    dt, Q = o.dtype, o.shape[0]
+    _chain_rows(dt, Q, o=o, x=x, qpos=qpos)
+    n = woffw.shape[0] * 16
+    _chain_weight(wo, dt, 256, 256, "wo"), _chain_weight(woffw, dt, n, 256, "woffw")
+    x2 = torch.empty((Q, 256), dtype=dt, device=o.device)
+    offw = torch.empty((Q, n), dtype=torch.float32, device=o.device)
+    ref_in, L = None, 0
+    if ref is not None:
+        if ref.dtype != torch.float32 or vr4.dtype != torch.float32 or not ref.is_contiguous() or not vr4.is_contiguous() or tuple(ref.shape) != (Q, 4):
+            raise TypeError("ape_amd.ops.dec_chain_c: ref [Q, 4] / vr4 [L, 4] must be contiguous float32")
+        L = vr4.shape[0]
+        ref_in = torch.empty((Q, L, 4), dtype=torch.float32, device=o.device)
+    rc = _lib.load().ape_hip_dec_chain_c(_p(o), _ld(o), _p(x), _ld(x), _p(qpos), _ld(qpos), Q, _DT[dt], _p(wo), _p(_f32vec(bo, "bo")),
+                                         _p(_f32vec(norm[0], "norm weight")), _p(_f32vec(norm[1], "norm bias")), float(norm[2]), _p(woffw),
+                                         _p(_f32vec(boffw, "boffw")), n, _p(x2), 256, _p(offw), n, _p(ref), _p(vr4), L, _p(ref_in), _stream())
+    _lib.check(rc, "ape_hip_dec_chain_c")
+    return (x2, offw) if ref is None else (x2, offw, ref_in)
+
+
+def dec_chain_t(samp, x2, qpos, wout, bout, norm1, w1, b1, w2, b2, norm2, *, box=None, ref=None, vr4=None, eps=1e-3):
+    _dev(samp, x2, qpos, wout, bout, w1, b1, w2, b2, norm1[0], norm1[1], norm2[0], norm2[1], ref, vr4)
+    dt, Q = samp.dtype, samp.shape[0]
+    _chain_rows(dt, Q, samp=samp, x2=x2, qpos=qpos)
+    hidden = w1.shape[0] * 16
+    _chain_weight(wout, dt, 256, 256, "wout"), _chain_weight(w1, dt, hidden, 256, "w1"), _chain_weight(w2, dt, 256, hidden, "w2")
+    out = torch.empty((Q, 256), dtype=dt, device=samp.device)
+    outp = torch.empty((Q, 256), dtype=dt, device=samp.device)
+    delta = new_ref = ref_in = None
+    bw = [None] * 6
+    L = 0
+    if box is not None:
+        (wb1, bb1), (wb2, bb2), (wb3, bb3) = box
+        _dev(wb1, bb1, wb2, bb2, wb3, bb3)
+        _chain_weight(wb1, dt, 256, 256, "box w1"), _chain_weight(wb2, dt, 256, 256, "box w2"), _chain_weight(wb3, dt, 4, 256, "box w3")
+        if ref.dtype != torch.float32 or vr4.dtype != torch.float32 or not ref.is_contiguous() or not vr4.is_contiguous() or tuple(ref.shape) != (Q, 4):
+            raise TypeError("ape_amd.ops.dec_chain_t: ref [Q, 4] / vr4 [L, 4] must be contiguous float32")
+        L = vr4.shape[0]
+        delta = torch.empty((Q, 4), dtype=torch.float32, device=samp.device)
+        new_ref = torch.empty((Q, 4), dtype=torch.float32, device=samp.device)
+        ref_in = torch.empty((Q, L, 4), dtype=torch.float32, device=samp.device)
+        bw = [_p(wb1), _p(_f32vec(bb1, "box b1")), _p(wb2), _p(_f32vec(bb2, "box b2")), _p(wb3), _p(_f32vec(bb3, "box b3"))]
+    rc = _lib.load().ape_hip_dec_chain_t(_p(samp), _ld(samp), _p(x2), _ld(x2), _p(qpos), _ld(qpos), Q, _DT[dt], _p(wout), _p(_f32vec(bout, "bout")),
+                                         _p(_f32vec(norm1[0], "norm1 weight")), _p(_f32vec(norm1[1], "norm1 bias")), float(norm1[2]), _p(w1),
+                                         _p(_f32vec(b1, "b1")), _p(w2), _p(_f32vec(b2, "b2")), hidden, _dec_chain_splitk(Q, hidden, dt),
+                                         _p(_f32vec(norm2[0], "norm2 weight")), _p(_f32vec(norm2[1], "norm2 bias")), float(norm2[2]), *bw,
+                                         _p(ref) if box is not None else None, _p(vr4) if box is not None else None, L, float(eps), _p(out), 256,
+                                         _p(outp), 256, _p(delta), _p(new_ref), _p(ref_in), _stream())
+    _lib.check(rc, "ape_hip_dec_chain_t")
+    return out, outp, delta, new_ref, ref_in
+
+
 def det_records(det_boxes, det_scores, det_classes, det_query, frame):
     _dev(det_boxes, det_scores, det_classes, det_query, frame)
     k = det_scores.numel()
diff --git a/ape_amd/packing.py b/ape_amd/packing.py
--- a/ape_amd/packing.py
+++ b/ape_amd/packing.py
@@ -12,6 +12,16 @@
     out = torch.zeros((Np, Kp), dtype=dtype, device=w.device)
     out[:N, :K] = w.detach().to(dtype)
     return out
+
+
+def pack_fragments(w):
+    N, K = w.shape
+    assert K % 32 == 0
+    Np = round_up(N, 16)
+    w = w.detach()
+    if Np != N:
+        w = torch.cat([w, w.new_zeros((Np - N, K))], 0)
+    return w.reshape(Np // 16, 16, K // 32, 4, 8).permute(0, 2, 3, 1, 4).contiguous().view(Np // 16, K // 32, 64, 8)
 
 
 def ffn_w2_perm(hid):
diff --git a/include/ape_hip.h b/include/ape_hip.h
--- a/include/ape_hip.h
+++ b/include/ape_hip.h
@@ -270,6 +270,17 @@
                        const double* det_area, const double* thresholds, int T, const double* ranges, int A, int* match,
                        uint8_t* flag, void* stream);
 
+int ape_hip_dec_chain_c(const void* o, int ldo, const void* x, int ldx, const void* qpos, int ldq, int Q, int dt, const void* wo,
+                        const float* bo, const float* ln_w, const float* ln_b, float eps, const void* woffw, const float* boffw,
+                        int noffw, void* x2, int ldx2, float* offw, int ldoffw, const float* ref, const float* vr4, int L,
+                        float* ref_in, void* stream);
+int ape_hip_dec_chain_t(const void* samp, int lds, const void* x2, int ldx2, const void* qpos, int ldq, int Q, int dt,
+                        const void* wout, const float* bout, const float* ln1_w, const float* ln1_b, float eps1, const void* w1,
+                        const float* b1, const void* w2, const float* b2, int hidden, int splitk, const float* ln2_w,
+                        const float* ln2_b, float eps2, const void* wb1, const float* bb1, const void* wb2, const float* bb2,
+                        const void* wb3, const float* bb3, const float* ref, const float* vr4, int L, float box_eps, void* out,
+                        int ldout, void* outp, int ldoutp, float* delta, float* new_ref, float* ref_in, void* stream);
+
 #ifdef __cplusplus
 }
 #endif
```

Measured after the change: 114.4. No clear change (-0.2%).
